# SamsungLabs/imvoxelnet

Hardware: AMD Instinct MI355X
Metric: images/sec/node (KITTI 3x384x1280, 216x248x12 vox) (higher is better)
Workload: dtype f32 (fp16 (hi, lo) pair MFMA operands: the Winograd-domain neck GEMMs and the chained 2-D trunk); 1 GPU; kitti_mono_1x3x384x1280_vox216x248x12_resnet50_fpn64_kittineck_anchor3dhead; batch_per_gpu=4, global_batch=4, parallelism=dp1, api=ImVoxelNet.simple_test(img, img_metas), detections_last_step=64

## Files before the change

imvoxelnet_amd/_lib.py:

```python
import ctypes as C
import os

_HERE = os.path.dirname(os.path.abspath(__file__))
LIB_PATH = os.environ.get('IVX_LIB_PATH') or os.path.join(_HERE, 'csrc', 'libimvoxel_hip.so')
_lib = None


class IvxError(RuntimeError):
    pass


class ConvDesc(C.Structure):
    _fields_ = [(n, C.c_int32) for n in
                ('B', 'D', 'H', 'W', 'Cin', 'Cout', 'KD', 'KH', 'KW', 'sd', 'sh', 'sw', 'pd', 'ph', 'pw',
                 'relu', 'res_mode', 'res_h', 'res_w', 'wgt_layout', 'out_mode', 'res_after_act')] + [('post_scale', C.c_float),
                                                                  ('in_dtype', C.c_int32), ('out_dtype', C.c_int32), ('res_scale', C.c_float),
                                                                  ('wino_operands', C.c_int32)]


class ConvRouteOpts(C.Structure):
    _fields_ = [(n, C.c_int32) for n in ('winograd', 'winograd_tile', 'wino_operands', 'split')] + [('winograd_min_pos', C.c_int64), ('winograd_2d_min_ch', C.c_int32)]


class ConvRoute(C.Structure):
# ... 66 lines not shown
                ('bytes', C.c_double), ('name', C.c_char * 48)]


class PlanInfo(C.Structure):
    _fields_ = [(n, C.c_int64) for n in ('cam_bytes', 'arena', 'ws_off', 'ws_bytes', 'ws2_off', 'ws2_bytes', 'total', 'scal_off', 'scal_bytes')] + \
               [(n, C.c_int32) for n in ('slot_bytes', 'n_sides', 's0', 's1', 'n_steps', 'n_tensors')]


class PlanStep(C.Structure):
    _fields_ = [(n, C.c_int32) for n in ('kind', 'in_', 'res', 'out', 'out2', 'fuse_out', 'fuse', 'side', 'join', 'tile', 'pio', 'amax_n', 'amax_in_n',
                                         'n_extra_in', 'n_extra_out')] + \
               [('extra_in', C.c_int32 * 12), ('extra_out', C.c_int32 * 4)] + \
               [(n, C.c_int64) for n in ('split', 'ws', 'amax_out', 'amax_in')] + [('name', C.c_char * 48)]


class PlanTensor(C.Structure):
    _fields_ = [(n, C.c_int64) for n in ('off', 'bytes', 'used', 'slot')] + \
               [(n, C.c_int32) for n in ('first', 'last', 'fmt', 'esz', 'caller_owned', 'boundary')]


class ImagePrepDesc(C.Structure):
    _fields_ = [(n, C.c_int32) for n in ('src_h', 'src_w', 'src_row_bytes', 'dst_h', 'dst_w', 'pad_h', 'pad_w', 'to_rgb')] + \
               [('mean', C.c_float * 3), ('std', C.c_float * 3)]


def declare_plan_view(L):
    key = [C.c_void_p, C.c_char_p, C.c_int32, C.c_int32, C.c_int32, C.c_int32]
    L.ivx_model_plan_info.argtypes = key + [C.POINTER(PlanInfo)]
    L.ivx_model_plan_step.argtypes = key + [C.c_int32, C.POINTER(PlanStep)]
    L.ivx_model_plan_tensor.argtypes = key + [C.c_int32, C.POINTER(PlanTensor)]


EXPORTS = ['ivx_model_plan_info', 'ivx_model_plan_step', 'ivx_model_plan_tensor', 'ivx_bottleneck_proj_supported', 'ivx_bottleneck_proj_pack', 'ivx_bottleneck_proj_fwd_pio', 'ivx_anchor_head_decode', 'ivx_fcos3d_head_decode', 'ivx_nms_rotated_bev', 'ivx_nms_aligned3d', 'ivx_bottleneck_supported', 'ivx_bottleneck_fwd_pio', 'ivx_amax_f32', 'ivx_stem_pool_filter_bytes', 'ivx_stem_pool_pack_filters', 'ivx_stem_pool_out_dims', 'ivx_stem_pool_fwd_pair', 'ivx_conv_winograd_set_variant', 'ivx_ubench_mfma', 'ivx_ubench_copy', 'ivx_version', 'ivx_last_error', 'ivx_conv_out_dims', 'ivx_conv_fwd', 'ivx_conv_fwd_naive', 'ivx_conv_set_tile_override', 'ivx_conv_set_epilogue_mode', 'ivx_conv_set_plan_mode', 'ivx_topk_set_mode', 'ivx_conv_workspace_bytes', 'ivx_conv_fwd_ws', 'ivx_conv_set_halo_mode', 'ivx_bf16_pair_split', 'ivx_f16_pair_split', 'ivx_conv_pair_supported', 'ivx_bf16_pair_pack_filters', 'ivx_conv_route', 'ivx_conv_pio_workspace_bytes', 'ivx_conv_fwd_pio', 'ivx_conv_fwd_pio_naive', 'ivx_pair_pack_filters', 'ivx_nchw_to_nhwc_amax', 'ivx_maxpool2d_fwd_pair', 'ivx_f16_pair_merge', 'ivx_model_calibrate_fp8', 'ivx_model_calibrate_fp8_ex', 'ivx_amax_bf16', 'ivx_conv_winograd_output_blocks', 'ivx_conv_winograd_issued_fraction', 'ivx_conv_winograd_output_amax', 'ivx_conv_winograd_input_amax', 'ivx_conv_winograd_fused_supported', 'ivx_conv_winograd_fused_blocks', 'ivx_conv_winograd_gemm_output_amax',
           'ivx_conv_winograd_supported', 'ivx_conv_winograd_weight_elems', 'ivx_conv_winograd_weights', 'ivx_conv_winograd_workspace_bytes',
           'ivx_conv_winograd_input', 'ivx_conv_winograd_gemm', 'ivx_conv_winograd_output', 'ivx_conv_winograd_fwd',
           'ivx_maxpool2d_fwd', 'ivx_maxpool2d_fwd_bf16', 'ivx_maxpool2d_fwd_fp8', 'ivx_global_avgpool_fwd', 'ivx_global_avgpool_fwd_bf16', 'ivx_upsample_trilinear2x_fwd', 'ivx_dcn_im2col_fwd', 'ivx_dcn_im2col_fwd_bf16', 'ivx_dcn_im2col_fwd_pair', 'ivx_nchw_to_nhwc', 'ivx_image_s2d_bf16', 'ivx_nhwc_to_nchw', 'ivx_backproject_mean_fwd', 'ivx_backproject_mean_fwd_amax', 'ivx_backproject_amax_blocks', 'ivx_backproject_mean_fwd_bf16', 'ivx_upsample_trilinear2x_fwd_bf16', 'ivx_backproject_sum_fwd', 'ivx_volume_normalize_fwd',
           'ivx_backproject_accum_fwd', 'ivx_backproject_accum_fwd_bf16', 'ivx_volume_mean_fwd', 'ivx_backproject_fwd_ex', 'ivx_backproject_gather_fwd',
           'ivx_anchor_head_workspace_bytes', 'ivx_anchor_head_get_bboxes', 'ivx_fcos_head_workspace_bytes',
           'ivx_fcos_head_level_candidates', 'ivx_nms_workspace_bytes',
           'ivx_nms_bev', 'ivx_boxes_overlap_bev', 'ivx_aligned_3d_nms', 'ivx_aligned_3d_nms_workspace_bytes', 'ivx_aligned_3d_nms_ws', 'ivx_multiclass_nms_workspace_bytes', 'ivx_multiclass_nms_bev',
           'ivx_create', 'ivx_destroy', 'ivx_weights_load', 'ivx_weights_finalize', 'ivx_model_workspace_bytes', 'ivx_model_forward',
           'ivx_backbone_fpn_workspace_bytes', 'ivx_backbone_fpn_fwd', 'ivx_neck3d_workspace_bytes', 'ivx_neck3d_out_dims',
           'ivx_neck3d_kitti_fwd', 'ivx_neck3d_nuscenes_fwd', 'ivx_neck3d_levels', 'ivx_neck3d_fast_fwd', 'ivx_neck3d_unet_fwd',
           'ivx_model_forward_levels', 'ivx_model_anchors', 'ivx_compute_projection', 'ivx_voxel_new_origin', 'ivx_fold_batchnorm',
           'ivx_model_trace', 'ivx_model_trace_count', 'ivx_model_trace_read',
           'ivx_model_detect_workspace_bytes', 'ivx_model_max_detections', 'ivx_model_detect', 'ivx_layout_head_decode', 'ivx_layout_extrinsics',
           'ivx_indoor_tail_workspace_bytes', 'ivx_indoor_tail_get_bboxes',
           'ivx_rescale_size', 'ivx_image_prep_u8',
           'ivx_kitti_image_box_overlap', 'ivx_kitti_compute_statistics', 'ivx_kitti_collect_scores', 'ivx_kitti_fused_statistics']


def lib():
    global _lib
    if _lib is not None:
        return _lib
    if not os.path.exists(LIB_PATH):
        raise IvxError(f'{LIB_PATH} is missing: build it with `python -m imvoxelnet_amd._build` '
                       '(or __graft_entry__.build()).  There is no CPU fallback.')
    L = C.CDLL(LIB_PATH)
    vp, i32, i64, f32 = C.c_void_p, C.c_int32, C.c_int64, C.c_float
    L.ivx_version.restype = C.c_int
    L.ivx_last_error.restype = C.c_char_p
    L.ivx_conv_out_dims.argtypes = [C.POINTER(ConvDesc), C.POINTER(i32), C.POINTER(i32), C.POINTER(i32)]
    for name in ('ivx_conv_fwd', 'ivx_conv_fwd_naive'):
        getattr(L, name).argtypes = [C.POINTER(ConvDesc), vp, vp, vp, vp, vp, vp, vp]
    L.ivx_conv_set_tile_override.argtypes = [C.c_int]
    L.ivx_conv_set_halo_mode.argtypes = [C.c_int]
    L.ivx_conv_set_epilogue_mode.argtypes = [C.c_int]
    L.ivx_conv_set_plan_mode.argtypes = [C.c_int]
    L.ivx_conv_winograd_output_blocks.argtypes = [C.POINTER(ConvDesc), i32]
    L.ivx_conv_winograd_output_blocks.restype = i32
    L.ivx_conv_winograd_output_amax.argtypes = [C.POINTER(ConvDesc), i32, vp, vp, vp, vp, vp, i64, vp, vp]
    L.ivx_conv_winograd_input_amax.argtypes = [C.POINTER(ConvDesc), i32, vp, vp, i64, vp, i32, vp]
    L.ivx_conv_winograd_fused_supported.argtypes = [C.POINTER(ConvDesc), i32]
    L.ivx_conv_winograd_fused_blocks.argtypes = [C.POINTER(ConvDesc), i32]
    L.ivx_conv_winograd_fused_blocks.restype = i32
    L.ivx_conv_winograd_gemm_output_amax.argtypes = [C.POINTER(ConvDesc), i32, vp, vp, vp, vp, vp, vp, i64, vp, vp]
    L.ivx_bf16_pair_split.argtypes = [vp, i64, vp, vp]
    L.ivx_f16_pair_split.argtypes = [vp, i64, f32, vp, vp]
    L.ivx_conv_pair_supported.argtypes = [C.POINTER(ConvDesc)]
    L.ivx_bf16_pair_pack_filters.argtypes = [vp, i32, i32, i32, i32, vp]
    L.ivx_conv_route.argtypes = [C.POINTER(ConvDesc), i32, C.POINTER(ConvRouteOpts), C.POINTER(ConvRoute)]
    L.ivx_conv_pio_workspace_bytes.argtypes = [C.POINTER(ConvDesc), C.POINTER(PairIO)]
    L.ivx_conv_pio_workspace_bytes.restype = i64
    L.ivx_amax_f32.argtypes = [vp, i64, vp, vp]
    L.ivx_stem_pool_filter_bytes.restype = i64
    L.ivx_stem_pool_filter_bytes.argtypes = []
    L.ivx_stem_pool_pack_filters.argtypes = [vp, vp, vp, vp]
    L.ivx_stem_pool_out_dims.argtypes = [i32, i32, C.POINTER(i32), C.POINTER(i32)]
    L.ivx_stem_pool_fwd_pair.argtypes = [vp, i32, i32, i32, vp, vp, vp, f32, f32, vp, vp, vp, vp, vp]
    L.ivx_bottleneck_supported.argtypes = [C.POINTER(BottleneckDesc)]
    L.ivx_bottleneck_fwd_pio.argtypes = [C.POINTER(BottleneckDesc), C.POINTER(BottleneckIO)] + [vp] * 12
    L.ivx_bottleneck_proj_supported.argtypes = [C.POINTER(BottleneckDesc), i32]
    L.ivx_bottleneck_proj_pack.argtypes = [vp, vp, vp, vp, vp, vp, i32, i32, vp, vp, vp, C.POINTER(f32), C.POINTER(f32), C.POINTER(f32)]
    L.ivx_bottleneck_proj_fwd_pio.argtypes = [C.POINTER(BottleneckDesc), i32, C.POINTER(BottleneckIO), f32] + [vp] * 12
    L.ivx_conv_fwd_pio.argtypes = [C.POINTER(ConvDesc), C.POINTER(PairIO), vp, vp, vp, vp, vp, vp, vp, i64, vp]
    L.ivx_conv_fwd_pio_naive.argtypes = [C.POINTER(ConvDesc), C.POINTER(PairIO), vp, vp, vp, vp, vp, vp, vp]
    L.ivx_pair_pack_filters.argtypes = [vp, i32, i32, i32, vp, vp, vp, vp, C.POINTER(f32), C.POINTER(f32)]
    L.ivx_nchw_to_nhwc_amax.argtypes = [vp, i32, i32, i64, i32, vp, vp, vp]
    L.ivx_maxpool2d_fwd_pair.argtypes = [vp, i32, i32, i32, i32, i32, i32, i32, vp, vp, f32, f32, vp, vp, vp]
    L.ivx_f16_pair_merge.argtypes = [vp, i64, vp, vp, vp]
    L.ivx_conv_workspace_bytes.argtypes = [C.POINTER(ConvDesc)]
    L.ivx_conv_workspace_bytes.restype = i64
    L.ivx_conv_fwd_ws.argtypes = [C.POINTER(ConvDesc), vp, vp, vp, vp, vp, vp, vp, i64, vp]
    D = C.POINTER(ConvDesc)
    L.ivx_conv_winograd_supported.argtypes = [D, i32]
    L.ivx_conv_winograd_issued_fraction.argtypes = [D]
    L.ivx_conv_winograd_issued_fraction.restype = C.c_float
    L.ivx_conv_winograd_weight_elems.argtypes = [D, i32]
    L.ivx_conv_winograd_weight_elems.restype = i64
# ... 107 lines not shown
```

imvoxelnet_amd/csrc/conv_igemm.hip:

```cpp
#include "ivx_common.h"
#include <stdlib.h>

#ifndef IVX_CONV_TU
#define IVX_CONV_TU 0
#endif
struct ConvParams;
struct ConvPlan;
int ivx_conv_launch_f32(ConvParams &p, const ConvPlan &pl, hipStream_t st);
int ivx_conv_launch_lowp(ConvParams &p, const ConvPlan &pl, hipStream_t st);
int ivx_conv_launch_pair_bf16(ConvParams &p, const ConvPlan &pl, hipStream_t st);
int ivx_conv_launch_pair_f16(ConvParams &p, const ConvPlan &pl, hipStream_t st);
int ivx_conv_launch_halo(ConvParams &p, int cfg, hipStream_t st);
int ivx_conv_launch_fold4(ConvParams &p, const IvxWinoFold &f, int n2, hipStream_t st);
int ivx_conv_fold4_blocks(long long M, int Cout);

typedef float f32x16 __attribute__((ext_vector_type(16)));
typedef float f32x4 __attribute__((ext_vector_type(4)));
typedef float f32x2 __attribute__((ext_vector_type(2)));
typedef __bf16 bf16x8 __attribute__((ext_vector_type(8)));
typedef _Float16 f16x8 __attribute__((ext_vector_type(8)));

struct ConvParams {
  const float *in, *wgt, *scale, *shift, *res;
  float *out;
  int B, D, H, W, Cin;
  int Cout, KD, KH, KW;
  int sd, sh, sw, pd, ph, pw;
  int Do, Ho, Wo;
  int M, K;
  int relu, res_mode, rH, rW;
  int kmode;
  int out_mode;
  int Cr;
  int res_after_act;
  float post_scale;
  int ksplit;
  float *partial;
  int q_total, q_begin, q_count, bm;
  int in_bf16;
  int out_bf16;
  long long g_in, g_w, g_out;
  int groups;
  int narrow_epilogue;
  int in_fp8;
  int out_fp8;
  float res_scale;
  int in_pair;
  int pio;
  const float *in_scale_p;
  int out_pair, res_pair;
  const float *res_scale_p;
  float *out_scale_p;
  const unsigned *amax_in, *amax_res;
  unsigned *amax_out;
  float wbound, sbound;
  const unsigned *cp_src;
  unsigned *cp_dst;
  int stagger_ticks, stagger_shift, stagger_first;
#ifdef IVX_CONV_TIMELINE
  unsigned long long *tl;
#endif
};

struct PairIO { float inv_in, inv_res, s_out; bool sat; float post; };
__device__ __forceinline__ PairIO conv_pair_io(const ConvParams &p) {
  PairIO io = {1.0f, 1.0f, 1.0f, false, p.post_scale};
  if (p.in_scale_p) io.inv_in = 1.0f / *p.in_scale_p;
  if (p.res_pair && p.res_scale_p) io.inv_res = 1.0f / *p.res_scale_p;
  if (p.out_pair) {
    const int lane = threadIdx.x & 63;
    float a = p.amax_in ? __uint_as_float(p.amax_in[lane]) : 0.f;
    float r = (p.amax_res && p.res_mode) ? __uint_as_float(p.amax_res[lane]) : 0.f;
#pragma unroll
    for (int o = 32; o > 0; o >>= 1) {
      a = fmaxf(a, __shfl_xor(a, o));
      r = fmaxf(r, __shfl_xor(r, o));
    }
    const float bound = (a * p.wbound + p.sbound + r) * fabsf(p.post_scale) * 1.001f;
    io.s_out = ivx_pow2_scale(bound);
    io.sat = !(bound < 3.0e38f);
    if (io.sat) io.s_out = 0.00390625f;
  }
  return io;
}
__device__ __forceinline__ size_t pair_off(size_t row, int n, int C) { return row * (size_t)(2 * C) + (size_t)((n >> 4) * 32 + (n & 15)); }

struct fp8_t { unsigned char v; };
typedef long i64_t;

__device__ __forceinline__ float fp8_to_f32(unsigned char b) { return __builtin_amdgcn_cvt_f32_fp8((int)b, 0); }
// ... 1166 lines not shown
    IVX_REQUIRE(!(d->res_mode && io->res_dtype == IVX_F16_PAIR) || (d->Cout % 16 == 0 && io->res_scale), "ivx_conv_fwd_pio: a pair residual needs Cout %% 16 == 0 and res_scale");
  }
  IVX_REQUIRE(!pair || (d->Cin % 16 == 0 && d->out_mode == 0), "ivx_conv_fwd: bf16-pair input needs Cin %% 16 == 0 and out_mode 0");
  IVX_REQUIRE(d->in_dtype != IVX_FP8 || d->Cin % 16 == 0, "ivx_conv_fwd: fp8 input needs Cin %% 16 == 0");
  IVX_REQUIRE((d->in_dtype != IVX_FP8 && d->out_dtype != IVX_FP8) || d->out_mode == 0, "ivx_conv_fwd: fp8 is built for out_mode 0 only");
  const int ck = d->in_dtype == IVX_FP8 ? 128 : (d->in_dtype == IVX_BF16 ? 64 : 32);
  IVX_REQUIRE(d->wgt_layout == 0 || (d->wgt_layout == 1 && d->Cin % ck == 0),
              "ivx_conv_fwd: wgt_layout 1 needs Cin %% %d == 0 (128-byte channel chunks)", ck);
  IVX_REQUIRE(d->in_dtype == IVX_F32 || d->Cin % 8 == 0, "ivx_conv_fwd: bf16 input needs Cin %% 8 == 0");
  IVX_REQUIRE(d->res_mode == 0 || res, "ivx_conv_fwd: res_mode set but res is NULL");
  if (d->res_mode == 2) {
    IVX_REQUIRE(Do == 1 && d->res_h > 0 && d->res_w > 0, "ivx_conv_fwd: res_mode 2 needs a 2-D output and res dims");
  }
  p->in = (const float *)in; p->wgt = (const float *)wgt; p->scale = scale; p->shift = shift;
  p->res = d->res_mode ? (const float *)res : nullptr; p->out = (float *)out;
  p->in_bf16 = d->in_dtype == IVX_BF16 || pair; p->out_bf16 = d->out_dtype == IVX_BF16;
  p->in_pair = d->in_dtype == IVX_BF16_PAIR ? 1 : (d->in_dtype == IVX_F16_PAIR ? 2 : 0);
  p->in_fp8 = d->in_dtype == IVX_FP8; p->out_fp8 = d->out_dtype == IVX_FP8;
  p->res_scale = d->res_scale == 0.f ? 1.0f : d->res_scale;
  p->B = d->B; p->D = d->D; p->H = d->H; p->W = d->W; p->Cin = cin_el;
  p->Cout = d->Cout; p->KD = d->KD; p->KH = d->KH; p->KW = d->KW;
  p->sd = d->sd; p->sh = d->sh; p->sw = d->sw; p->pd = d->pd; p->ph = d->ph; p->pw = d->pw;
  p->Do = Do; p->Ho = Ho; p->Wo = Wo; p->M = (int)M; p->K = (int)K;
  p->relu = d->relu; p->res_mode = d->res_mode; p->rH = d->res_h; p->rW = d->res_w; p->kmode = d->wgt_layout;
  p->out_mode = d->out_mode; p->Cr = d->out_mode == 1 ? d->Cout / 8 : d->Cout; p->res_after_act = d->res_after_act;
  p->post_scale = d->post_scale == 0.f ? 1.0f : d->post_scale;
  p->ksplit = 1; p->partial = nullptr; p->q_total = 0; p->q_begin = 0; p->q_count = 0; p->bm = 0;
  p->stagger_ticks = 0; p->stagger_shift = 0; p->stagger_first = 0;
  p->groups = 1; p->g_in = p->g_w = p->g_out = 0;
  p->narrow_epilogue = g_narrow_epilogue;
#ifdef IVX_CONV_TIMELINE
  p->tl = g_timeline;
#endif
  p->cp_src = nullptr; p->cp_dst = nullptr;
  p->pio = 0; p->in_scale_p = nullptr; p->out_pair = 0; p->res_pair = 0; p->res_scale_p = nullptr; p->out_scale_p = nullptr;
  p->amax_in = p->amax_res = nullptr; p->amax_out = nullptr; p->wbound = 0.f; p->sbound = 0.f;
  if (io) {
    p->pio = 1;
    p->in_scale_p = io->in_scale;
    p->out_pair = d->out_dtype == IVX_F16_PAIR; p->out_bf16 = 0;
    p->res_pair = d->res_mode && io->res_dtype == IVX_F16_PAIR;
    p->res_scale_p = io->res_scale; p->out_scale_p = p->out_pair ? io->out_scale : nullptr;
    p->amax_in = io->amax_in; p->amax_res = d->res_mode ? io->amax_res : nullptr; p->amax_out = io->amax_out;
    p->wbound = io->wbound; p->sbound = io->sbound;
  }
  return IVX_OK;
}

extern "C" int ivx_conv_out_dims(const ivx_conv_desc *d, int32_t *Do, int32_t *Ho, int32_t *Wo) {
  IVX_REQUIRE(d && Do && Ho && Wo, "ivx_conv_out_dims: null argument");
  const int od = (d->D + 2 * d->pd - d->KD) / d->sd + 1;
  const int oh = (d->H + 2 * d->ph - d->KH) / d->sh + 1;
  const int ow = (d->W + 2 * d->pw - d->KW) / d->sw + 1;
  IVX_REQUIRE(d->D + 2 * d->pd >= d->KD && d->H + 2 * d->ph >= d->KH && d->W + 2 * d->pw >= d->KW && od > 0 && oh > 0 && ow > 0,
              "ivx_conv_out_dims: kernel larger than padded input");
  *Do = od; *Ho = oh; *Wo = ow;
  return IVX_OK;
}

template <int TM, int TN, int WR, int WC>
static void launch_cfg(const ConvParams &p, hipStream_t st) {
  constexpr int BM = WR * TM * 32, BN = WC * TN * 32;
  dim3 grid((p.M + BM - 1) / BM, (p.Cout + BN - 1) / BN);
  hipLaunchKernelGGL((conv_igemm_f32_kernel<TM, TN, WR, WC>), grid, dim3(256), 0, st, p);
}

#endif
// ... 285 lines not shown
      ivx_set_error("ivx_conv_fwd: tile %d has no pair-operand instantiation (61, 63, 66, 67, 73 .. 77, 81 .. 83, 85, 166, 174, 177, 179, 183; fp16 pairs also 474, 475, 574)", pl.cfg);
      return IVX_ERR_INVALID_ARG;
  }
  return IVX_OK;
}

#if IVX_CONV_TU == 3
int ivx_conv_launch_pair_bf16(ConvParams &p, const ConvPlan &pl, hipStream_t st) { return launch_pair<1>(p, pl, st); }
#else
int ivx_conv_launch_pair_f16(ConvParams &p, const ConvPlan &pl, hipStream_t st) { return launch_pair<2>(p, pl, st); }
#endif
#endif

#if IVX_CONV_TU == 5
template <typename T, int TM, int TN, int WR, int WC, int WPE, int PAIR, int NBUF, int TAIL = 1, int SW = 1, int ZR = 0, int DI = 0>
__global__ __launch_bounds__(64 * WR * WC, WPE) void conv_wino_halo_kernel(const ConvParams p, const unsigned in_bytes, const unsigned w_bytes) {
  constexpr int BM = WR * TM * 32, BN = WC * TN * 32, NT = 64 * WR * WC;
  constexpr int BK = 32, EPC = 8, NCH = 4, RP = NT / NCH;
  static_assert((SW * BM) % RP == 0 && (3 * BN) % RP == 0, "A rows and the three taps of B rows in whole passes (+ one 16-row tail pass of A)");
  static_assert(SW == 1 || TAIL == 0, "the stride-2 form uses overlapping tiles");
  static_assert(!DI || SW == 2, "de-interleaved staging is the stride-2 form's");
  constexpr int APASS = SW * BM / RP, AROWS = SW * BM + 16 * TAIL;
  constexpr int BMO = TAIL ? BM : (SW == 1 ? BM - 2 - ZR : BM - 1);
  constexpr int ZROW = TAIL ? BM + 2 : SW * BM - 1;
  constexpr int BPASS = 3 * BN / RP;
  constexpr int BUF = (AROWS + 3 * BN) * BK;
  constexpr int D = NBUF - 1;
  constexpr int LPG = APASS + BPASS;
  static_assert((D - 1) * (LPG + TAIL) <= 15, "vmcnt immediate");
  __shared__ __attribute__((aligned(16))) T smem[NBUF * BUF];
  static_assert(sizeof(smem) >= (size_t)NT / 64 * 4096, "4 KB of staging LDS per wave for the transposed epilogue");
  const int tid = threadIdx.x, lane = tid & 63, wid = tid >> 6;
  const int wr = wid / WC, wc = wid % WC;
  int mt, nt;
  {
    const int Nt = (p.Cout + BN - 1) / BN;
    const int xcd = blockIdx.x & 7, idx = blockIdx.x >> 3;
    const int lt = idx / Nt;
    nt = idx - lt * Nt;
    mt = xcd * p.q_total + lt;
  }
  if (mt * BMO >= p.M) return;
  const int m0 = mt * BMO, n0 = nt * BN;
  const size_t gz = blockIdx.z;
  if (p.cp_dst && blockIdx.x == 0 && blockIdx.z == 0 && tid == 0) *p.cp_dst = *p.cp_src;
#ifdef IVX_CONV_TIMELINE
  const unsigned long long tl0 = __builtin_amdgcn_s_memrealtime();
  unsigned long long tl1 = 0, tl2 = 0;
#endif
  const __amdgpu_buffer_rsrc_t rs_in =
      __builtin_amdgcn_make_buffer_rsrc((void *)((const char *)p.in + gz * (size_t)p.g_in * sizeof(T)), 0, in_bytes, 0x00020000);
  const __amdgpu_buffer_rsrc_t rs_w =
      __builtin_amdgcn_make_buffer_rsrc((void *)((const char *)p.wgt + gz * (size_t)p.g_w * sizeof(T)), 0, w_bytes, 0x00020000);
  const int lr = tid / NCH;
  const int cc = (tid & (NCH - 1)) ^ ((lr >> 2) & 3);
  const int wid_u = __builtin_amdgcn_readfirstlane(wid);
  const unsigned OOB = 0x80000000u;
  typedef __attribute__((address_space(3))) void *lds_ptr_t;
  unsigned a_base[APASS + 1];
  a_base[APASS] = OOB;
#pragma unroll
  for (int j = 0; j < APASS + TAIL; ++j) {
    const int li = j < APASS ? lr + RP * j : BM + (lane >> 2);
    const int row = SW * m0 - 1 + (DI ? (li < BM ? 2 * li : 2 * (li - BM) + 1) : li);
    const bool zr = ZR && !TAIL && li == ZROW;
    a_base[j] = (row >= 0 && row < SW * p.M && (j < APASS || (lane >> 2) < 2) && !zr) ? ((unsigned)row * (unsigned)p.Cin + cc * EPC) * (unsigned)sizeof(T) : OOB;
  }
  unsigned b_base[BPASS];
#pragma unroll
  for (int j = 0; j < BPASS; ++j) {
    const int r = lr + RP * j, tap = r / BN, n = n0 + (r - tap * BN);
    b_base[j] = n < p.Cout ? ((unsigned)n * (unsigned)p.K + tap * 64 + cc * EPC) * (unsigned)sizeof(T) : OOB;
  }
  const int G = p.Cin / BK;
  auto load_group = [&](int g, int buf) {
    T *Ab = smem + buf * BUF + wid_u * (64 / NCH) * BK;
    T *Bb = Ab + AROWS * BK;
    const unsigned ka = (unsigned)g * BK * (unsigned)sizeof(T);
    const unsigned kb = ((unsigned)(g >> 1) * 3u * 64u + (unsigned)(g & 1) * 32u) * (unsigned)sizeof(T);
#pragma unroll
    for (int j = 0; j < APASS; ++j) {
      const unsigned vo = a_base[j] == OOB ? OOB : a_base[j] + ka;
      __builtin_amdgcn_raw_ptr_buffer_load_lds(rs_in, (lds_ptr_t)(Ab + RP * j * BK), 16, vo, 0, 0, 0);
    }
    if (TAIL && wid_u == 0) {
      const unsigned vo = a_base[APASS] == OOB ? OOB : a_base[APASS] + ka;
      __builtin_amdgcn_raw_ptr_buffer_load_lds(rs_in, (lds_ptr_t)(smem + buf * BUF + BM * BK), 16, vo, 0, 0, 0);
    }
#pragma unroll
    for (int j = 0; j < BPASS; ++j) {
      const unsigned vo = b_base[j] == OOB ? OOB : b_base[j] + kb;
      __builtin_amdgcn_raw_ptr_buffer_load_lds(rs_w, (lds_ptr_t)(Bb + RP * j * BK), 16, vo, 0, 0, 0);
    }
  };
  const int rl = lane & 31, fh = lane >> 5;
  bool ok0[TM], ok2[TM];
#pragma unroll
  for (int i = 0; i < TM; ++i) {
    const int z = (m0 + (wr * TM + i) * 32 + rl) % p.Wo;
// ... 65 lines not shown
        const T *rowp = Bc + (kz * BN + j * 32 + rl) * BK;
        bh[j] = *reinterpret_cast<const f32x4 *>(rowp + ((fh ^ bsw) * EPC));
        bl[j] = *reinterpret_cast<const f32x4 *>(rowp + (((2 + fh) ^ bsw) * EPC));
      }
      if (!ZR && kz != 1) {
#pragma unroll
        for (int i = 0; i < TM; ++i) {
          const bool ok = kz == 0 ? ok0[i] : ok2[i];
          ah[i] = ok ? ah[i] : zero4;
          al[i] = ok ? al[i] : zero4;
        }
      }
#pragma unroll
      for (int i = 0; i < TM; ++i)
#pragma unroll
        for (int j = 0; j < TN; ++j) {
          acc[i][j] = pair_mfma<PAIR>(ah[i], bh[j], acc[i][j]);
          acc[i][j] = pair_mfma<PAIR>(ah[i], bl[j], acc[i][j]);
          acc[i][j] = pair_mfma<PAIR>(al[i], bh[j], acc[i][j]);
        }
    }
    cur = cur + 1 == NBUF ? 0 : cur + 1;
    nxt = nxt + 1 == NBUF ? 0 : nxt + 1;
  }
#ifdef IVX_CONV_TIMELINE
  tl2 = __builtin_amdgcn_s_memrealtime();
#endif
  __syncthreads();
  if constexpr (TAIL) {
    conv_epilogue_wide<TM, TN>(p, acc, m0, n0, wr, wc, lane, reinterpret_cast<float *>(smem) + wid_u * 1024, gz * (size_t)p.g_out);
  } else {
    float *stage = reinterpret_cast<float *>(smem) + wid_u * 1024;
    float *outp = p.out + gz * (size_t)p.g_out;
    const int mlim = (m0 + BMO < p.M) ? m0 + BMO : p.M;
    const int col_l = lane & 31, hh = lane >> 5, rrow = lane >> 3, c4 = (lane & 7) * 4;
#pragma unroll
    for (int j = 0; j < TN; ++j) {
      const int nb = n0 + (wc * TN + j) * 32 + c4;
      const bool nok = nb < p.Cout;
#pragma unroll
      for (int i = 0; i < TM; ++i) {
#pragma unroll
        for (int r = 0; r < 16; ++r) stage[((r & 3) + 8 * (r >> 2) + 4 * hh) * 32 + col_l] = acc[i][j][r];
        const int mb = m0 + (wr * TM + i) * 32 + rrow;
#pragma unroll
        for (int q = 0; q < 4; ++q) {
          const f32x4 v = *reinterpret_cast<const f32x4 *>(stage + (rrow + 8 * q) * 32 + c4);
          const int m = mb + 8 * q;
          if (m < mlim && nok) *reinterpret_cast<f32x4 *>(outp + (size_t)m * p.Cout + nb) = v;
        }
      }
    }
  }
#ifdef IVX_CONV_TIMELINE
  if (p.tl && tid == 0) {
    unsigned long long *t = p.tl + ((size_t)blockIdx.z * gridDim.x + blockIdx.x) * 8;
    t[0] = tl0; t[1] = tl1; t[2] = tl2; t[3] = __builtin_amdgcn_s_memrealtime();
    t[4] = __builtin_amdgcn_s_getreg(63492); t[5] = __builtin_amdgcn_s_getreg(63508);
  }
#endif
}

template <int TM, int TN, int WR, int WC, int WPE, int PAIR, int NBUF, int TAIL = 1, int SW = 1, int ZR = 0, int DI = 0>
static void launch_halo(ConvParams &p, hipStream_t st) {
  constexpr int BM = (WR * TM * 32) - (TAIL ? 0 : (SW == 1 ? 2 + ZR : 1)), BN = WC * TN * 32;
  const int64_t in_bytes = (int64_t)p.B * p.D * p.H * p.W * p.Cin * 2, w_bytes = (int64_t)p.Cout * p.K * 2;
  const long long Mt = (p.M + BM - 1) / BM, Nt = (p.Cout + BN - 1) / BN;
  p.bm = BM;
  p.q_total = (int)((Mt + 7) / 8); p.q_begin = 0; p.q_count = p.q_total;
  const dim3 grid((unsigned)(8LL * p.q_total * Nt), 1, p.groups > 1 ? p.groups : 1);
  auto kern = conv_wino_halo_kernel<__bf16, TM, TN, WR, WC, WPE, PAIR, NBUF, TAIL, SW, ZR, DI>;
  hipLaunchKernelGGL(kern, grid, dim3(64 * WR * WC), 0, st, p, (unsigned)in_bytes, (unsigned)w_bytes);
}

template <typename T, int Z, int WCOL, int WN, int WPE, int PAIR, int SW = 1>
__global__ __launch_bounds__(64 * WCOL * (Z / 3) * WN, WPE) void conv_wino_zblk_kernel(const ConvParams p, const unsigned in_bytes, const unsigned w_bytes) {
  static_assert(Z == 3 || Z == 6, "three output z-blocks per wave");
  constexpr int ZI = SW * Z;
  constexpr int ZH = Z / 3, NW = WCOL * ZH * WN, NT = 64 * NW;
  constexpr int CT = WCOL * 32, AR = ZI * CT, BN = WN * 32;
  constexpr int NS = 2 * SW + 3;
  constexpr int BK = 32, EPC = 8, NCH = 4, RP = NT / NCH;
  constexpr int APASS = (AR + RP - 1) / RP, BPASS = (3 * BN + RP - 1) / RP;
  static_assert(AR % 16 == 0 && (3 * BN) % 16 == 0, "a wave's 16 rows of a pass are inside or outside as a whole");
  constexpr int BUF = (AR + 3 * BN) * BK;
  __shared__ __attribute__((aligned(16))) T smem[2 * BUF];
  static_assert(sizeof(smem) >= (size_t)NW * 4096, "4 KB of staging LDS per wave for the transposed epilogue");
  const int tid = threadIdx.x, lane = tid & 63, wid = tid >> 6;
  const int wid_u = __builtin_amdgcn_readfirstlane(wid);
  const int cg = wid_u / (ZH * WN), zh = (wid_u / WN) % ZH, nb = wid_u % WN;
  int mt, nt;
  {
    const int Nt = (p.Cout + BN - 1) / BN;
    const int xcd = blockIdx.x & 7, idx = blockIdx.x >> 3;
    const int lt = idx / Nt;
    nt = idx - lt * Nt;
    mt = xcd * p.q_total + lt;
  }
  const int c0 = mt * CT, n0 = nt * BN;
  const int m0 = c0 * Z;
  if (m0 >= p.M) return;
#ifdef IVX_CONV_TIMELINE
  const unsigned long long tl0 = __builtin_amdgcn_s_memrealtime();
  unsigned long long tl1 = 0, tl2 = 0;
#endif
  const size_t gz = blockIdx.z;
  if (p.cp_dst && blockIdx.x == 0 && blockIdx.z == 0 && tid == 0) *p.cp_dst = *p.cp_src;
  const __amdgpu_buffer_rsrc_t rs_in =
      __builtin_amdgcn_make_buffer_rsrc((void *)((const char *)p.in + gz * (size_t)p.g_in * sizeof(T)), 0, in_bytes, 0x00020000);
  const __amdgpu_buffer_rsrc_t rs_w =
      __builtin_amdgcn_make_buffer_rsrc((void *)((const char *)p.wgt + gz * (size_t)p.g_w * sizeof(T)), 0, w_bytes, 0x00020000);
  const int lr = tid / NCH;
  const int cc = (tid & (NCH - 1)) ^ ((lr >> 2) & 3);
  const unsigned OOB = 0x80000000u;
  typedef __attribute__((address_space(3))) void *lds_ptr_t;
  unsigned a_base[APASS], b_base[BPASS];
#pragma unroll
  for (int j = 0; j < APASS; ++j) {
    const int li = lr + RP * j;
    const int z = li / CT, c = li - z * CT;
    const int row = (c0 + c) * ZI + z;
    a_base[j] = (li < AR && row < SW * p.M) ? ((unsigned)row * (unsigned)p.Cin + cc * EPC) * (unsigned)sizeof(T) : OOB;
  }
#pragma unroll
  for (int j = 0; j < BPASS; ++j) {
    const int r = lr + RP * j, tap = r / BN, n = n0 + (r - tap * BN);
    b_base[j] = (r < 3 * BN && n < p.Cout) ? ((unsigned)n * (unsigned)p.K + tap * 64 + cc * EPC) * (unsigned)sizeof(T) : OOB;
  }
  const int G = p.Cin / BK;
  auto load_group = [&](int g, int buf) {
    T *Ab = smem + buf * BUF + wid_u * (64 / NCH) * BK;
    T *Bb = Ab + AR * BK;
    const unsigned ka = (unsigned)g * BK * (unsigned)sizeof(T);
    const unsigned kb = ((unsigned)(g >> 1) * 3u * 64u + (unsigned)(g & 1) * 32u) * (unsigned)sizeof(T);
#pragma unroll
    for (int j = 0; j < APASS; ++j) {
      if (RP * j + wid_u * 16 < AR) {
        const unsigned vo = a_base[j] == OOB ? OOB : a_base[j] + ka;
        __builtin_amdgcn_raw_ptr_buffer_load_lds(rs_in, (lds_ptr_t)(Ab + RP * j * BK), 16, vo, 0, 0, 0);
      }
    }
#pragma unroll
    for (int j = 0; j < BPASS; ++j) {
      if (RP * j + wid_u * 16 < 3 * BN) {
        const unsigned vo = b_base[j] == OOB ? OOB : b_base[j] + kb;
        __builtin_amdgcn_raw_ptr_buffer_load_lds(rs_w, (lds_ptr_t)(Bb + RP * j * BK), 16, vo, 0, 0, 0);
      }
    }
  };
  const int rl = lane & 31, fh = lane >> 5, sw = (rl >> 2) & 3;
  const int z0 = zh * 3;
  f32x16 acc[3];
#pragma unroll
  for (int i = 0; i < 3; ++i)
#pragma unroll
// ... 23 lines not shown
    for (int kz = 0; kz < 3; ++kz) {
      const T *rowp = B0 + kz * BN * BK;
      const f32x4 bh = *reinterpret_cast<const f32x4 *>(rowp + ((fh ^ sw) * EPC));
      const f32x4 bl = *reinterpret_cast<const f32x4 *>(rowp + (((2 + fh) ^ sw) * EPC));
#pragma unroll
      for (int zo = 0; zo < 3; ++zo) {
        const int zs = SW * (z0 + zo) + kz - 1;
        if (zs >= 0 && zs < ZI) {
          acc[zo] = pair_mfma<PAIR>(ah[SW * zo + kz], bh, acc[zo]);
          acc[zo] = pair_mfma<PAIR>(ah[SW * zo + kz], bl, acc[zo]);
          acc[zo] = pair_mfma<PAIR>(al[SW * zo + kz], bh, acc[zo]);
        }
      }
    }
    cur ^= 1;
  }
#ifdef IVX_CONV_TIMELINE
  tl2 = __builtin_amdgcn_s_memrealtime();
#endif
  __syncthreads();
  float *stage = reinterpret_cast<float *>(smem) + wid_u * 1024;
  float *outp = p.out + gz * (size_t)p.g_out;
  const int col_l = lane & 31, hh = lane >> 5, rrow = lane >> 3, c4 = (lane & 7) * 4;
  const int nbc = n0 + nb * 32 + c4;
  const bool nok = nbc < p.Cout;
#pragma unroll
  for (int zo = 0; zo < 3; ++zo) {
#pragma unroll
    for (int r = 0; r < 16; ++r) stage[((r & 3) + 8 * (r >> 2) + 4 * hh) * 32 + col_l] = acc[zo][r];
#pragma unroll
    for (int q = 0; q < 4; ++q) {
      const f32x4 v = *reinterpret_cast<const f32x4 *>(stage + (rrow + 8 * q) * 32 + c4);
      const int m = m0 + (cg * 32 + rrow + 8 * q) * Z + z0 + zo;
      if (m < p.M && nok) *reinterpret_cast<f32x4 *>(outp + (size_t)m * p.Cout + nbc) = v;
    }
  }
#ifdef IVX_CONV_TIMELINE
  if (p.tl && tid == 0) {
    unsigned long long *t = p.tl + ((size_t)blockIdx.z * gridDim.x + blockIdx.x) * 8;
    t[0] = tl0; t[1] = tl1; t[2] = tl2; t[3] = __builtin_amdgcn_s_memrealtime();
    t[4] = __builtin_amdgcn_s_getreg(63492); t[5] = __builtin_amdgcn_s_getreg(63508);
  }
#endif
}

template <int Z, int WCOL, int WN, int WPE, int SW = 1>
static void launch_zblk(ConvParams &p, hipStream_t st) {
  constexpr int AR = Z * WCOL * 32, BN = WN * 32;
  const int64_t in_bytes = (int64_t)p.B * p.D * p.H * p.W * p.Cin * 2, w_bytes = (int64_t)p.Cout * p.K * 2;
  const long long Mt = (p.M + AR - 1) / AR, Nt = (p.Cout + BN - 1) / BN;
  p.bm = AR;
  p.q_total = (int)((Mt + 7) / 8); p.q_begin = 0; p.q_count = p.q_total;
  const dim3 grid((unsigned)(8LL * p.q_total * Nt), 1, p.groups > 1 ? p.groups : 1);
  auto kern = conv_wino_zblk_kernel<__bf16, Z, WCOL, WN, WPE, 2, SW>;
  hipLaunchKernelGGL(kern, grid, dim3(64 * WCOL * (Z / 3) * WN), 0, st, p, (unsigned)in_bytes, (unsigned)w_bytes);
}

static int zblk_wrong_z(int want, int got) {
  ivx_set_error("ivx_conv_launch_halo: this z-blocked config is built for columns of %d slices, the layer has %d", want, got);
  return IVX_ERR_INVALID_ARG;
}

int ivx_conv_launch_halo(ConvParams &p, int cfg, hipStream_t st) {
  if (p.in_pair != 2) {
    ivx_set_error("ivx_conv_launch_halo: fp16 pair operands only");
    return IVX_ERR_INVALID_ARG;
  }
// ... 485 lines not shown
    if (!launch) continue;
    if (pl.ws_bytes > 0 && (!workspace || workspace_bytes < pl.ws_bytes)) {
      ivx_set_error("%s: workspace too small (%lld < %lld); size it with ivx_conv_workspace_bytes", who, (long long)workspace_bytes,
                    (long long)pl.ws_bytes);
      return IVX_ERR_WORKSPACE;
    }
    const int rc = run_conv(q, pl, workspace, st);
    if (rc != IVX_OK) return rc;
  }
  return IVX_OK;
}

extern "C" int ivx_conv_fwd(const ivx_conv_desc *d, const void *in, const void *wgt, const float *scale,
                            const float *shift, const void *res, void *out, ivx_stream_t stream) {
  ConvParams p;
  int rc = fill_params(d, in, wgt, scale, shift, res, out, &p);
  if (rc != IVX_OK) return rc;
  int64_t need;
  rc = conv_dispatch(p, false, true, nullptr, 0, (hipStream_t)stream, &need, "ivx_conv_fwd");
  if (rc != IVX_OK) return rc;
  IVX_CHECK_LAUNCH("ivx_conv_fwd");
  return IVX_OK;
}

static bool zblk_rule(const ConvParams &p) { return p.Wo == 3 && p.W == 3 && p.Cout > 64; }

extern "C" float ivx_conv_winograd_issued_fraction(const ivx_conv_desc *d) {
  if (!d || d->wino_operands != IVX_F16_PAIR || d->KW != 3 || d->sw != 1 || d->pw != 1 || d->W != 3 || d->Cin % 64 || d->Cout <= 64 || d->wgt_layout != 1 ||
      g_halo_mode >= 0 || g_tile_override != 0)
    return 1.0f;
  return 7.0f / 9.0f;
}

int ivx_conv_grouped_launch(const ivx_conv_desc *d, int groups, const float *in, long long g_in, const float *wgt, long long g_w,
                            float *out, long long g_out, hipStream_t st, const unsigned *cp_src, unsigned *cp_dst) {
  ConvParams p;
  int rc = fill_params(d, in, wgt, nullptr, nullptr, nullptr, out, &p);
  if (rc != IVX_OK) return rc;
  IVX_REQUIRE(groups >= 1 && groups <= 65535, "ivx_conv_grouped_launch: bad group count");
  IVX_REQUIRE((d->in_dtype == IVX_F32 || d->in_dtype == IVX_BF16_PAIR || d->in_dtype == IVX_F16_PAIR) && d->out_dtype == IVX_F32 &&
                  d->out_mode == 0 && d->res_mode == 0,
              "ivx_conv_grouped_launch: fp32 or pair operands, plain fp32 output only");
  if (!dma_applicable(p)) {
    ivx_set_error("ivx_conv_grouped_launch: one group must stay below 2 GiB");
    return IVX_ERR_UNSUPPORTED;
  }
  if (cp_dst && !p.in_pair) {
    if (hipMemcpyAsync(cp_dst, cp_src, 4, hipMemcpyDeviceToDevice, st) != hipSuccess) {
      ivx_set_error("ivx_conv_grouped_launch: hipMemcpyAsync failed");
      return IVX_ERR_HIP;
    }
  } else {
    p.cp_src = cp_src; p.cp_dst = cp_dst;
  }
  p.groups = groups; p.g_in = g_in; p.g_w = g_w; p.g_out = g_out;
  if (p.in_pair == 2 && p.kmode == 1 && d->KD == 1 && d->KH == 1 && d->KW == 3 && d->sw == 2 && d->pw == 1 && p.W == 2 * p.Wo && p.Cin % 64 == 0 &&
      ((g_halo_mode >= 21 && g_halo_mode < 30) || (g_halo_mode >= 40 && g_halo_mode < 50) || g_halo_mode >= 70 || (g_halo_mode < 0 && g_tile_override == 0))) {
    return ivx_conv_launch_halo(p, g_halo_mode >= 21 ? g_halo_mode : 42, st);
  }
  if (p.in_pair == 2 && p.kmode == 1 && d->KD == 1 && d->KH == 1 && d->KW == 3 && d->sw == 1 && d->pw == 1 && p.Cin % 64 == 0 &&
      ((g_halo_mode > 0 && g_halo_mode < 21) || (g_halo_mode >= 30 && g_halo_mode < 40) || (g_halo_mode >= 50 && g_halo_mode < 70) ||
       (g_halo_mode < 0 && g_tile_override == 0))) {
    static const int halo_small = getenv("IVX_HALO_SMALL") ? atoi(getenv("IVX_HALO_SMALL")) : 1;
    const bool few = halo_small && p.Cout > 64 && !zblk_rule(p) && (long long)((p.M + 252) / 253) * ((p.Cout + 127) / 128) * groups < 512;
    const int cfg = g_halo_mode > 0 ? g_halo_mode : ((p.Cout <= 64 || few) ? 30 : (zblk_rule(p) ? 50 : 33));
    return ivx_conv_launch_halo(p, cfg, st);
  }
  ConvPlan pl = {g_tile_override, 1, 1, 0, 0, 0, 0};
  if (pl.cfg == 0 && p.in_pair) {
    pl.cfg = p.Cout <= 64 ? 76 : (p.Cout <= 128 ? 81 : (p.in_pair == 2 && p.kmode == 1 ? 183 : 82));
    const long long nblk = (long long)groups * ((p.M + 127) / 128) * ((p.Cout + 127) / 128);
    if (nblk < 2500) pl.cfg = 67;
  }
  if (pl.cfg == 0) {
    const long long nblk = (long long)groups * ((p.M + 127) / 128) * ((p.Cout + 127) / 128);
    if (p.Cout <= 32) pl.cfg = 44;
    else if (nblk >= 2500) pl.cfg = p.Cout > 64 ? (p.Cout == 128 && p.K == 384 ? 58 : 54) : 49;
    else pl.cfg = p.K <= 640 ? 47 : 46;
  }
  TileInfo t;
  if (!tile_info(pl.cfg, &t) || (pl.cfg >= 61) != (p.in_pair != 0)) {
    ivx_set_error("ivx_conv_grouped_launch: tile %d does not match the operand type", pl.cfg);
    return IVX_ERR_INVALID_ARG;
  }
  return launch_one(p, pl, st);
}

int ivx_conv_grouped_fold4(const ivx_conv_desc *d, int groups, const float *in, long long g_in, const float *wgt, long long g_w, const IvxWinoFold *f,
                           hipStream_t st) {
  ConvParams p;
  float dummy;
  int rc = fill_params(d, in, wgt, nullptr, nullptr, nullptr, &dummy, &p);
  if (rc != IVX_OK) return rc;
  IVX_REQUIRE(d->in_dtype == IVX_F16_PAIR && d->KD == 1 && d->KH == 1 && d->KW == 3 && d->sw == 1 && d->pw == 1 && d->wgt_layout == 1 && f && f->out,
              "ivx_conv_grouped_fold4: fp16 pair operands, 1x1x3 along z with stride 1 and padding 1, chunk-major filters");
  p.groups = groups; p.g_in = g_in; p.g_w = g_w; p.g_out = 0;
  return ivx_conv_launch_fold4(p, *f, groups, st);
}

// ... 81 lines not shown
```

imvoxelnet_amd/csrc/model.cpp:

```cpp
#include <hip/hip_runtime_api.h>
#include <math.h>
#include <stdarg.h>
#include <string.h>

#include <algorithm>
#include <cstdlib>
#include <map>
#include <memory>
#include <string>
#include <vector>

#include "../../include/imvoxel.h"
#include "../../include/imvoxel_lab.h"

void ivx_set_error(const char *fmt, ...);

#define M_REQUIRE(cond, ...)        \
  do {                              \
    if (!(cond)) {                  \
      ivx_set_error(__VA_ARGS__);   \
      return IVX_ERR_INVALID_ARG;   \
    }                               \
  } while (0)
#define M_HIP(call, what)                                                        \
  do {                                                                           \
    hipError_t e_ = (call);                                                      \
    if (e_ != hipSuccess) {                                                      \
      ivx_set_error("%s: %s", what, hipGetErrorString(e_));                      \
      return IVX_ERR_HIP;                                                        \
    }                                                                            \
  } while (0)
#define M_TRY(call)                 \
  do {                              \
    int rc_ = (call);               \
    if (rc_ != IVX_OK) return rc_;  \
  } while (0)

namespace {

inline int64_t align256(int64_t v) { return (v + 255) / 256 * 256; }

inline uint16_t f32_to_f16_bits(float f) {
  uint32_t x;
  memcpy(&x, &f, 4);
  const uint32_t sign = (x >> 16) & 0x8000u, ax = x & 0x7fffffffu;
  if (ax >= 0x7f800000u) return (uint16_t)(sign | (ax > 0x7f800000u ? 0x7e00u : 0x7c00u));
  if (ax < 0x38800000u) {
    float a;
// ... 78 lines not shown

struct Step {
  StepKind kind;
  int layer = -1;
  int in = -1, res = -1, out = -1, out2 = -1;
  int res_mode = 0;
  int res_after_act = 0;
  float post_scale = 1.0f;
  int aux = 0;
};

struct TInfo {
  int B = 0, D = 0, H = 0, W = 0, C = 0;
  int64_t bytes = 0, off = -1;
  int first = -1, last = -1;
  bool raw = false;
  int esz = 4;
  int fmt = 0;
  int64_t slot = -1;
  int64_t elems() const { return (int64_t)B * D * H * W * C; }
};

struct PlanStep {
  ivx_conv_desc d;
  int tile = 0;
  int64_t ws = 0;
  int64_t amax_out = -1, amax_in = -1;
  int amax_n = 0, amax_in_n = 0;
  int pio = 0;
  int64_t split = 0;
  int bound_layer = -1;
  int fuse = 0, fuse_out = -1;
  int side = 0, join = 0;
};

struct Plan {
  std::vector<TInfo> t;
  std::vector<PlanStep> ps;
  int64_t arena = 0, ws_off = 0, ws_bytes = 0, tail_ws = 0, total = 0;
  ivx_anchor_head_desc tail;
  int64_t cam_bytes = 0, cam_proj = 0, cam_origin = 0, cam_crop = 0, cam_lvl_vs[3] = {0, 0, 0}, cam_lvl_no[3] = {0, 0, 0};
  int n_views = 1;
  ivx_indoor_tail_desc itail;
  int max_det = 0;
  int64_t scal_off = 0, scal_bytes = 0;
  int64_t ws2_off = 0, ws2_bytes = 0;
  int n_sides = 0;
  int s0 = 0, s1 = 0;
};

}

struct ivx_model {
  ivx_model_cfg cfg;
  std::vector<ConvLayer> layers;
  std::vector<Step> steps;
  int n_tensors = 0;
  int trunk0 = 0, trunk1 = 0, lift_step = -1, neck0 = 0, neck1 = 0, head_step = -1, tail_step = -1;
  int t_img = -1, t_fpn0 = -1, t_volume = -1, t_valid = -1, t_neck = -1, t_head = -1;
  std::vector<int> t_levels;
  int head0 = -1;
  std::vector<int> t_headout, t_cb, t_cs, t_cc;
  float head_scales[3] = {1.f, 1.f, 1.f};
  int t_c5 = -1, t_angle = -1, t_layout = -1, layout_step = -1;
  std::vector<std::vector<char>> cam_ring;
  size_t cam_next = 0;
  std::map<std::string, HostTensor> weights;
  bool finalized = false;
  std::vector<float> anchors_host;
  int anchors_h = 0, anchors_w = 0;
  float *anchors_dev = nullptr;
  size_t anchors_cap = 0;
  std::vector<float> anchors_given;
  std::map<std::string, std::unique_ptr<Plan>> plans;
  std::vector<void *> owned;
  std::vector<float> pack_a, pack_b;
  bool fp8_on = false;
  float *calib_dev = nullptr;
  bool trace_on = false;
  bool trace_skip = false;
  int trace_level = 2;
  struct TraceRec { int step, stage, is3d; double flops, bytes; hipEvent_t e0, e1; std::string name; };
  std::vector<TraceRec> trace;
  std::vector<hipEvent_t> event_pool;
  size_t events_used = 0;
  hipStream_t side = nullptr;
  hipEvent_t ev_fork = nullptr;
  std::vector<hipEvent_t> ev_join;
};

namespace {

int new_tensor(ivx_model *m) { return m->n_tensors++; }

int add_conv(ivx_model *m, ConvLayer L, int in, int res = -1, int res_mode = 0) {
  m->layers.push_back(std::move(L));
  Step s;
  s.kind = ST_CONV;
  s.layer = (int)m->layers.size() - 1;
  s.in = in;
  s.res = res;
  s.res_mode = res >= 0 ? (res_mode ? res_mode : 1) : 0;
  s.out = new_tensor(m);
  m->steps.push_back(s);
  return s.out;
}

ConvLayer conv2d(const std::string &name, int cin, int cout, int k, int stride, int pad, bool relu, const std::string &w,
                 const std::string &b, const std::string &bn) {
  ConvLayer L;
  L.name = name; L.dims = 2; L.cin = cin; L.cout = cout;
  L.k[0] = 1; L.k[1] = k; L.k[2] = k;
  L.s[0] = 1; L.s[1] = stride; L.s[2] = stride;
  L.p[0] = 0; L.p[1] = pad; L.p[2] = pad;
  L.relu = relu; L.w_keys = {w}; L.b_keys = {b}; L.bn = bn;
// ... 884 lines not shown
    }
  }
  for (int i = r.s0; i < r.s1; ++i) {
    const Step &s = m->steps[i];
    PlanStep &pc = pl->ps[i];
    if (s.kind != ST_CONV || pc.tile == 0 || pc.d.wino_operands != IVX_F16_PAIR) continue;
    for (int j = i - 1; j >= r.s0; --j) {
      const Step &q = m->steps[j];
      if (q.out != s.in) continue;
      PlanStep &pp = pl->ps[j];
      if (q.kind == ST_LIFT && m->cfg.sampling == IVX_SAMPLE_NEAREST) {
        const TInfo &vol = pl->t[q.out];
        const int32_t nb = ivx_backproject_amax_blocks(vol.B, n_views, vol.D, vol.H, vol.W);
        if (nb > 0) {
          if (pp.amax_out < 0) { pp.amax_out = top; pp.amax_n = nb; top += align256((int64_t)nb * 4); }
          pc.amax_in = pp.amax_out;
          pc.amax_in_n = pp.amax_n;
        }
      }
      if (q.kind == ST_CONV && pp.tile > 0) {
        if (pp.amax_out < 0) {
          const int32_t nb = ivx_conv_winograd_output_blocks(&pp.d, pp.tile);
          M_REQUIRE(nb > 0, "layer %s: %s", m->layers[q.layer].name.c_str(), ivx_last_error());
          pp.amax_out = top;
          pp.amax_n = nb;
          top += align256((int64_t)nb * 4);
        }
        pc.amax_in = pp.amax_out;
        pc.amax_in_n = pp.amax_n;
      }
      break;
    }
  }
  if (n_slots > 0) {
    top = align256(top);
    pl->scal_off = top;
    pl->scal_bytes = (int64_t)n_slots * 512;
    top += pl->scal_bytes;
  }
  pl->arena = align256(top);
  pl->ws_off = pl->arena;
  pl->ws_bytes = align256(pl->ws_bytes);
  pl->total = pl->arena + pl->ws_bytes;
  if (pl->n_sides > 0) {
    for (int i = r.s0; i < r.s1; ++i)
      if (pl->ps[i].side > 0) pl->ws2_bytes = std::max(pl->ws2_bytes, pl->ps[i].ws);
    pl->ws2_bytes = align256(pl->ws2_bytes);
    pl->ws2_off = pl->total;
    pl->total += pl->ws2_bytes;
  }
  return IVX_OK;
}

std::string plan_key(const char *what, int B, int V, int H, int W) {
  char buf[96];
  snprintf(buf, sizeof(buf), "%s:%d:%d:%d:%d", what, B, V, H, W);
  return buf;
}

TInfo tinfo(int B, int D, int H, int W, int C, int esz = 4) {
  TInfo t; t.B = B; t.D = D; t.H = H; t.W = W; t.C = C; t.esz = esz; t.bytes = align256(t.elems() * esz);
  return t;
}

int get_plan(ivx_model *m, const char *what, Range r, int B, int V, int H, int W, const std::map<int, TInfo> &inputs, Plan **out,
             hipStream_t stream) {
// ... 64 lines not shown
  }
  if (!m->anchors_dev) {
    void *p = nullptr;
    M_HIP(hipMalloc(&p, std::max<size_t>(n, 1) * sizeof(float)), "hipMalloc (anchors)");
    m->owned.push_back(p);
    m->anchors_dev = (float *)p;
    m->anchors_cap = n;
  }
  M_HIP(hipMemcpyAsync(m->anchors_dev, m->anchors_host.data(), n * sizeof(float), hipMemcpyHostToDevice, st), "hipMemcpyAsync (anchors)");
  M_HIP(hipStreamSynchronize(st), "hipStreamSynchronize (anchors)");
  m->anchors_h = d.H; m->anchors_w = d.W;
  return IVX_OK;
}

int run_steps(ivx_model *m, const Plan &pl, Range r, const Bind &bd, void *workspace, int64_t workspace_bytes, hipStream_t st,
              const char *who) {
  M_REQUIRE(workspace && ((uintptr_t)workspace & 255) == 0, "%s: workspace must be non-null and 256-byte aligned", who);
  if (workspace_bytes < pl.total) {
    ivx_set_error("%s: workspace too small (%lld < %lld); size it with the matching *_workspace_bytes call", who, (long long)workspace_bytes,
                  (long long)pl.total);
    return IVX_ERR_WORKSPACE;
  }
  char *base = (char *)workspace;
  void *ws = base + pl.ws_off;
  auto ptr = [&](int t) -> void * {
    auto it = bd.ext.find(t);
    if (it != bd.ext.end()) return it->second;
    return base + pl.t[t].off;
  };
  auto slotp = [&](int t) -> uint32_t * { return (t >= 0 && pl.t[t].slot >= 0) ? (uint32_t *)(base + pl.scal_off + pl.t[t].slot * 512) : nullptr; };
  auto scalep = [&](int t) -> float * { uint32_t *q = slotp(t); return q ? (float *)(q + IVX_AMAX_SLOTS) : nullptr; };
  if (pl.scal_bytes > 0 && r.s0 <= m->trunk0 && r.s1 > m->trunk0)
    M_HIP(hipMemsetAsync(base + pl.scal_off, 0, (size_t)pl.scal_bytes, st), "hipMemsetAsync (amax slots)");
  const bool span2d = m->trace_on && m->trace_level == 1 && m->cfg.with_trunk;
  std::vector<char> forked((size_t)std::max(pl.n_sides, 1), 0);
  double span_flops = 0.0, span_bytes = 0.0;
  for (int i = r.s0; i < r.s1; ++i) {
    const Step &s = m->steps[i];
    const TInfo &in = pl.t[s.in];
    const bool in_span = span2d && i >= m->trunk0 && i < m->trunk1;
    if (in_span && i == m->trunk0) M_TRY(trace_begin(m, i, 6, 0, 0.0, 0.0, "2-D trunk (ResNet-50 + FPN level 0)", st));
    const bool was_on = m->trace_on;
    if (in_span) {
      m->trace_on = false;
      {
        const PlanStep &ps = pl.ps[i];
        auto tb = [&](int t) { return t >= 0 ? (double)pl.t[t].elems() * pl.t[t].esz : 0.0; };
        if (s.kind == ST_CONV && ps.fuse != 2) {
          const ConvLayer &L = m->layers[s.layer];
          if (ps.fuse == 1) {
            const ConvLayer &L2 = m->layers[m->steps[i + 1].layer], &L3 = m->layers[m->steps[i + 2].layer];
            span_bytes += tb(s.in) + tb(ps.fuse_out) + 4.0 * ((double)L.cout * L.cin + 9.0 * L2.cout * L2.cin + (double)L3.cout * L3.cin);
          } else if (ps.fuse == 5) {
            const ConvLayer &L2 = m->layers[m->steps[i + 1].layer], &L3 = m->layers[m->steps[i + 2].layer];
            span_bytes += tb(s.in) + tb(ps.fuse_out) + 4.0 * ((double)L.cout * L.cin + 9.0 * L2.cout * L2.cin + (double)L3.cout * (L3.cin + L.cin));
          } else {
            span_bytes += tb(s.in) + tb(s.out) + tb(s.res) + (double)pl.t[s.in].esz * L.cout * L.cin_pad * L.k[0] * L.k[1] * L.k[2];
          }
        } else if (s.kind == ST_MAXPOOL && ps.fuse == 4) {
          span_bytes += tb(s.out) + tb(m->t_img);
        } else if (s.kind == ST_IMG2CL && ps.fuse == 3) {
          span_bytes += tb(s.in);
        } else if (s.kind != ST_CONV && s.kind != ST_LAYOUT) {
          span_bytes += tb(s.in) + tb(s.out) + tb(s.res);
        }
      }
// ... 102 lines not shown
        const void *res = s.res >= 0 ? ptr(s.res) : nullptr;
        const TInfo &o = pl.t[s.out];
        const int is3d = in.D > 1 && in.W > 1;
        hipStream_t cst = st;
        void *cws = ws;
        int64_t cws_bytes = pl.ws_bytes;
        if (ps.side > 0 && !(m->trace_on && m->trace_level != 3) && pl.ws2_off > 0) {
          if (!m->side) {
            M_HIP(hipStreamCreateWithFlags(&m->side, hipStreamNonBlocking), "hipStreamCreateWithFlags");
            M_HIP(hipEventCreateWithFlags(&m->ev_fork, hipEventDisableTiming), "hipEventCreateWithFlags");
          }
          while ((int)m->ev_join.size() < pl.n_sides) {
            hipEvent_t e;
            M_HIP(hipEventCreateWithFlags(&e, hipEventDisableTiming), "hipEventCreateWithFlags");
            m->ev_join.push_back(e);
          }
          M_HIP(hipEventRecord(m->ev_fork, st), "hipEventRecord");
          M_HIP(hipStreamWaitEvent(m->side, m->ev_fork, 0), "hipStreamWaitEvent");
          cst = m->side;
          cws = base + pl.ws2_off;
          cws_bytes = pl.ws2_bytes;
          forked[ps.side - 1] = 1;
        }
        if (ps.join > 0 && forked[ps.join - 1]) {
          M_HIP(hipStreamWaitEvent(st, m->ev_join[ps.join - 1], 0), "hipStreamWaitEvent");
          forked[ps.join - 1] = 0;
        }
        if (ps.tile && m->trace_on) {
          const int n = ps.tile + 2, tiles = o.B * ((ps.d.D + 2 * ps.d.pd - 2 + ps.tile - 1) / ps.tile) * ((ps.d.H + 2 * ps.d.ph - 2 + ps.tile - 1) / ps.tile);
          int32_t zo_d, zo_h, zo;
          M_TRY(ivx_conv_out_dims(&ps.d, &zo_d, &zo_h, &zo));
          const double vb = 4.0 * n * n * tiles * ps.d.W * ps.d.Cin, mb = 4.0 * n * n * tiles * zo * ps.d.Cout;
          M_TRY(trace_begin(m, i, 1, is3d, 0.0, 4.0 * in.elems() + vb, L.name, st));
          M_TRY(ivx_conv_winograd_input_amax(&ps.d, ps.tile, ptr(s.in), ws, pl.ws_bytes, ps.amax_in >= 0 ? (const float *)(base + ps.amax_in) : nullptr,
                                             ps.amax_in_n, st));
          M_TRY(trace_end(m, st));
          M_TRY(trace_begin(m, i, 2, is3d, (ps.d.wino_operands ? 3.0 : 1.0) * ivx_conv_winograd_issued_fraction(&ps.d) * 2.0 * n * n * tiles * zo * ps.d.Cout * ps.d.KW * ps.d.Cin,
                            vb + mb, L.name, st));
          M_TRY(ivx_conv_winograd_gemm(&ps.d, ps.tile, L.u.at(ps.tile * 8 + ps.d.wino_operands), ws, pl.ws_bytes, st));
          M_TRY(trace_end(m, st));
          M_TRY(trace_begin(m, i, 3, is3d, 0.0, mb + 4.0 * o.elems() * (res ? 2 : 1), L.name, st));
          M_TRY(ivx_conv_winograd_output_amax(&ps.d, ps.tile, L.scale, L.shift, res, ptr(s.out), ws, pl.ws_bytes,
                                              ps.amax_out >= 0 ? (float *)(base + ps.amax_out) : nullptr, st));
          M_TRY(trace_end(m, st));
          break;
        }
        M_TRY(trace_begin(m, i, 0, is3d, ((ps.pio || ps.split) ? 3.0 : 1.0) * 2.0 * o.elems() * L.cin * L.k[0] * L.k[1] * L.k[2], 0.0, L.name, st));
        if (ps.pio) {
          ivx_pair_io io;
          memset(&io, 0, sizeof(io));
          io.in_scale = scalep(s.in);
          io.res_dtype = s.res >= 0 ? pl.t[s.res].fmt : 0;
          io.res_scale = io.res_dtype == IVX_F16_PAIR ? scalep(s.res) : nullptr;
          io.out_scale = scalep(s.out);
          io.amax_in = slotp(s.in); io.amax_res = slotp(s.res); io.amax_out = slotp(s.out);
          io.wbound = L.wbound; io.sbound = L.sbound;
          M_TRY(ivx_conv_fwd_pio(&ps.d, &io, ptr(s.in), L.wpair, L.scale_p, L.shift, res, ptr(s.out), cws, cws_bytes, cst));
        } else if (ps.tile) {
          M_TRY(ivx_conv_winograd_input_amax(&ps.d, ps.tile, ptr(s.in), ws, pl.ws_bytes, ps.amax_in >= 0 ? (const float *)(base + ps.amax_in) : nullptr,
                                             ps.amax_in_n, st));
          M_TRY(ivx_conv_winograd_gemm(&ps.d, ps.tile, L.u.at(ps.tile * 8 + ps.d.wino_operands), ws, pl.ws_bytes, st));
          M_TRY(ivx_conv_winograd_output_amax(&ps.d, ps.tile, L.scale, L.shift, res, ptr(s.out), ws, pl.ws_bytes,
                                              ps.amax_out >= 0 ? (float *)(base + ps.amax_out) : nullptr, st));
        } else if (m->fp8_on && L.fp8_eff) {
          M_TRY(ivx_conv_fwd_ws(&ps.d, ptr(s.in), L.fp8_eff >= 2 ? L.wq : L.w, L.scale_q, L.shift_q, res, ptr(s.out), cws, cws_bytes, cst));
        } else if (ps.split) {
          M_TRY(ivx_bf16_pair_split((const float *)ptr(s.in), in.elems(), cws, cst));
          M_TRY(ivx_conv_fwd_ws(&ps.d, cws, L.wsplit, L.scale, L.shift, res, ptr(s.out), (char *)cws + ps.split, cws_bytes - ps.split, cst));
        } else {
          M_TRY(ivx_conv_fwd_ws(&ps.d, ptr(s.in), L.w, L.scale, L.shift, res, ptr(s.out), cws, cws_bytes, cst));
          if (m->calib_dev && (L.fp8_eff == 1 || L.fp8_eff == 2))
            M_TRY(ivx_amax_bf16(ptr(s.out), o.elems(), m->calib_dev + s.layer, st));
        }
        M_TRY(trace_end(m, st));
        if (cst != st) M_HIP(hipEventRecord(m->ev_join[ps.side - 1], cst), "hipEventRecord");
        break;
      }
      case ST_LIFT: {
        M_REQUIRE(bd.proj && bd.new_origin && bd.crop, "%s: proj / new_origin / crop_hw are required", who);
        const TInfo &o = pl.t[s.out];
        M_TRY(trace_begin(m, i, 4, 1, 0.0, (double)in.esz * in.elems() + (double)o.esz * o.elems() + (double)o.elems() / o.C, "unprojection", st));
        if (m->cfg.sampling != IVX_SAMPLE_NEAREST) {
          ivx_backproject_desc ld = {};
          ld.B = o.B; ld.V = bd.V; ld.FH = in.H; ld.FW = in.W; ld.C = in.C; ld.X = o.D; ld.Y = o.H; ld.Z = o.W;
          for (int a = 0; a < 3; ++a) ld.voxel_size[a] = m->cfg.voxel_size[a];
          ld.feat_dtype = m->cfg.storage == IVX_BF16 ? IVX_BF16 : IVX_F32;
          ld.mode = IVX_LIFT_MEAN;
          ld.sampling = m->cfg.sampling;
          M_TRY(ivx_backproject_fwd_ex(&ld, ptr(s.in), bd.proj, bd.new_origin, bd.crop, ptr(s.out), nullptr, nullptr, (uint8_t *)ptr(s.out2), st));
          M_TRY(trace_end(m, st));
          break;
        }
        if (m->cfg.storage == IVX_BF16) {
          if (bd.V == 1 && in.C % 8 == 0)
            M_TRY(ivx_backproject_mean_fwd((const float *)ptr(s.in), o.B, 1, in.H, in.W, in.C / 2, bd.proj, bd.new_origin, bd.crop, m->cfg.voxel_size, o.D,
                                           o.H, o.W, (float *)ptr(s.out), (uint8_t *)ptr(s.out2), st));
          else
            M_TRY(ivx_backproject_mean_fwd_bf16(ptr(s.in), o.B, bd.V, in.H, in.W, in.C, bd.proj, bd.new_origin, bd.crop, m->cfg.voxel_size, o.D, o.H, o.W,
                                                ptr(s.out), (uint8_t *)ptr(s.out2), st));
          M_TRY(trace_end(m, st));
          break;
        }
        M_TRY(ivx_backproject_mean_fwd_amax((const float *)ptr(s.in), o.B, bd.V, in.H, in.W, in.C, bd.proj, bd.new_origin, bd.crop, m->cfg.voxel_size,
                                            o.D, o.H, o.W, (float *)ptr(s.out), (uint8_t *)ptr(s.out2),
                                            pl.ps[i].amax_out >= 0 ? (float *)(base + pl.ps[i].amax_out) : nullptr, st));
        M_TRY(trace_end(m, st));
        break;
      }
      case ST_DCN_COL: {
        const TInfo &om = pl.t[s.res];
        M_TRY(trace_begin(m, i, 0, 0, 0.0, (double)pl.t[s.out].esz * pl.t[s.out].elems(), "dcn columns", st));
        if (pl.ps[i].pio)
          M_TRY(ivx_dcn_im2col_fwd_pair(ptr(s.in), scalep(s.in), (const float *)ptr(s.res), in.B, in.H, in.W, in.C, 3, 3, s.aux, 1, 1, om.C,
                                        ptr(s.out), scalep(s.out), slotp(s.out), st));
        else if (m->cfg.storage == IVX_BF16)
          M_TRY(ivx_dcn_im2col_fwd_bf16(ptr(s.in), (const float *)ptr(s.res), in.B, in.H, in.W, in.C, 3, 3, s.aux, 1, 1, om.C, ptr(s.out), st));
        else
          M_TRY(ivx_dcn_im2col_fwd((const float *)ptr(s.in), (const float *)ptr(s.res), in.B, in.H, in.W, in.C, 3, 3, s.aux, 1, 1, om.C,
                                   (float *)ptr(s.out), st));
        M_TRY(trace_end(m, st));
        break;
      }
      case ST_AVGPOOL:
        if (m->cfg.storage == IVX_BF16)
          M_TRY(ivx_global_avgpool_fwd_bf16(ptr(s.in), in.B, (int64_t)in.D * in.H * in.W, in.C, (float *)ptr(s.out), st));
        else
          M_TRY(ivx_global_avgpool_fwd((const float *)ptr(s.in), in.B, (int64_t)in.D * in.H * in.W, in.C, (float *)ptr(s.out), st));
        break;
      case ST_LAYOUT: {
        if (!bd.metas && r.s1 == m->trunk1) break;
        M_REQUIRE(bd.metas && bd.proj_dev, "%s: a handle with a LayoutHead runs through ivx_model_detect (the projection is built from its angles)", who);
        const int B = in.B;
        std::vector<float> a((size_t)B * 2), l((size_t)B * 7), pj((size_t)B * 12);
        M_HIP(hipMemcpyAsync(a.data(), ptr(s.in), a.size() * 4, hipMemcpyDeviceToHost, st), "hipMemcpyAsync (angles)");
        M_HIP(hipMemcpyAsync(l.data(), ptr(s.res), l.size() * 4, hipMemcpyDeviceToHost, st), "hipMemcpyAsync (layout)");
        M_HIP(hipStreamSynchronize(st), "hipStreamSynchronize (LayoutHead)");
        for (int b = 0; b < B; ++b) {
          float ang[2], E[16];
          M_TRY(ivx_layout_head_decode(&a[(size_t)b * 2], &l[(size_t)b * 7], ang, bd.layout_host ? bd.layout_host + (size_t)b * 7 : nullptr));
// ... 586 lines not shown
        proj[(size_t)v * 12 + i * 4 + j] = acc;
      }
  }
  return IVX_OK;
}

extern "C" int ivx_voxel_new_origin(const float *origin, const int32_t *n_voxels, const float *voxel_size, float *new_origin) {
  M_REQUIRE(origin && n_voxels && voxel_size && new_origin, "ivx_voxel_new_origin: null argument");
  for (int a = 0; a < 3; ++a) {
    const float half = (float)n_voxels[a] / 2.0f;
    const float ext = half * voxel_size[a];
    new_origin[a] = origin[a] - ext;
  }
  return IVX_OK;
}

extern "C" int ivx_model_trace(ivx_model *m, int32_t enable) {
  M_REQUIRE(m, "ivx_model_trace: null handle");
  m->trace.clear();
  m->events_used = 0;
  m->trace_on = enable != 0;
  if (enable >= 1 && enable <= 3) m->trace_level = enable;
  return IVX_OK;
}

extern "C" int32_t ivx_model_trace_count(ivx_model *m) { return m ? (int32_t)m->trace.size() : -1; }

extern "C" int ivx_model_trace_read(ivx_model *m, int32_t i, ivx_trace_rec *rec) {
  M_REQUIRE(m && rec && i >= 0 && i < (int32_t)m->trace.size(), "ivx_model_trace_read: bad index");
  const ivx_model::TraceRec &r = m->trace[i];
  float ms = 0.f, start = 0.f;
  M_HIP(hipEventElapsedTime(&ms, r.e0, r.e1), "hipEventElapsedTime (synchronise the stream first)");
  M_HIP(hipEventElapsedTime(&start, m->trace[0].e0, r.e0), "hipEventElapsedTime");
  rec->step = r.step; rec->stage = r.stage; rec->is3d = r.is3d; rec->ms = ms; rec->start_ms = start; rec->flops = r.flops; rec->bytes = r.bytes;
  snprintf(rec->name, sizeof(rec->name), "%s", r.name.c_str());
  return IVX_OK;
}

static int plan_lookup(ivx_model *m, const char *what, int B, int V, int H, int W, const char *who, const Plan **pl) {
  M_REQUIRE(m && what, "%s: null argument", who);
  auto it = m->plans.find(plan_key(what, B, V, H, W));
  M_REQUIRE(it != m->plans.end(), "%s: no cached plan \"%s\" for (%d, %d, %d, %d); call the matching *_workspace_bytes first", who, what, B, V, H, W);
  *pl = it->second.get();
  return IVX_OK;
}

extern "C" int ivx_model_plan_info(ivx_model *m, const char *what, int32_t B, int32_t V, int32_t H, int32_t W, ivx_plan_info *info) {
  const Plan *pl;
  M_TRY(plan_lookup(m, what, B, V, H, W, "ivx_model_plan_info", &pl));
  M_REQUIRE(info, "ivx_model_plan_info: null argument");
  memset(info, 0, sizeof(*info));
  info->cam_bytes = pl->cam_bytes; info->arena = pl->arena; info->ws_off = pl->ws_off; info->ws_bytes = pl->ws_bytes;
  info->ws2_off = pl->ws2_off; info->ws2_bytes = pl->ws2_bytes; info->total = pl->total;
  info->scal_off = pl->scal_off; info->scal_bytes = pl->scal_bytes; info->slot_bytes = 512;
  info->n_sides = pl->n_sides; info->s0 = pl->s0; info->s1 = pl->s1;
  info->n_steps = (int32_t)m->steps.size(); info->n_tensors = m->n_tensors;
  return IVX_OK;
}

extern "C" int ivx_model_plan_step(ivx_model *m, const char *what, int32_t B, int32_t V, int32_t H, int32_t W, int32_t step, ivx_plan_step *rec) {
  const Plan *pl;
  M_TRY(plan_lookup(m, what, B, V, H, W, "ivx_model_plan_step", &pl));
  M_REQUIRE(rec && step >= pl->s0 && step < pl->s1, "ivx_model_plan_step: step %d is outside the plan's range [%d, %d)", step, pl->s0, pl->s1);
  const Step &s = m->steps[step];
  const PlanStep &ps = pl->ps[step];
  memset(rec, 0, sizeof(*rec));
  rec->kind = (int32_t)s.kind;
// ... 150 lines not shown
```

imvoxelnet_amd/csrc/winograd.hip:

```cpp
#include "ivx_common.h"
#include <stdlib.h>
int ivx_conv_launch_fold4w(const _Float16 *V, long long vs, const _Float16 *U, long long us, int M, int Cin_stored, int Cout, int Z, const IvxWinoFold &f,
                           hipStream_t st);

int ivx_conv_grouped_launch(const ivx_conv_desc *d, int groups, const float *in, long long g_in, const float *wgt, long long g_w,
                            float *out, long long g_out, hipStream_t st, const unsigned *cp_src, unsigned *cp_dst);
int ivx_conv_grouped_fold4(const ivx_conv_desc *d, int groups, const float *in, long long g_in, const float *wgt, long long g_w, const IvxWinoFold *f,
                           hipStream_t st);
int ivx_conv_fold4_blocks(long long M, int Cout);

namespace {

struct WinoP {
  const float *in, *scale, *shift, *res;
  float *out;
  float *V, *Mw;
  long long vs, ms;
  int B, X, Y, Z, C;
  int Xo, Yo, Zo, Co;
  int TX, TY;
  int px, py;
  int relu, res_mode, res_after_act;
  float post_scale;
  float *pmax;
  const unsigned *hdr;
#ifdef IVX_CONV_TIMELINE
  unsigned long long *tl;
#endif
};
#ifdef IVX_CONV_TIMELINE
#define WINO_TL_BEGIN const unsigned long long wtl0 = __builtin_amdgcn_s_memrealtime();
#define WINO_TL_END(p)                                                                                              \
  if ((p).tl && threadIdx.x == 0) {                                                                                \
    unsigned long long *t_ = (p).tl + (size_t)blockIdx.x * 8;                                                       \
    t_[0] = wtl0; t_[1] = wtl0; t_[2] = wtl0; t_[3] = __builtin_amdgcn_s_memrealtime();                             \
    t_[4] = __builtin_amdgcn_s_getreg(63492); t_[5] = __builtin_amdgcn_s_getreg(63508);                             \
  }
#else
#define WINO_TL_BEGIN
#define WINO_TL_END(p)
#endif

__device__ __forceinline__ bool wino_amax_bad(const float amax) { return !(amax < 3.0e38f); }
__device__ __forceinline__ float wino_pow2_scale(const float amax, const float gain_log2) {
  if (wino_amax_bad(amax)) return 0.00390625f;
  if (!(amax > 0.f)) return 1.0f;
  int e;
  (void)frexpf(amax, &e);
  int k = 15 - (int)gain_log2 - e;
  k = k < -120 ? -120 : (k > 120 ? 120 : k);
  return ldexpf(1.0f, k);
}
__device__ __forceinline__ float wino_pair_vscale(const unsigned *hdr) { return wino_pow2_scale(__uint_as_float(hdr[0]), 8.f); }
__device__ __forceinline__ float wino_mscale(const unsigned *hdr) { return hdr ? 1.0f / (wino_pair_vscale(hdr) * __uint_as_float(hdr[1])) : 1.0f; }

__device__ __forceinline__ float vabsmax(const float v) { return fabsf(v); }
__device__ __forceinline__ float vabsmax(const float2 v) { return fmaxf(fabsf(v.x), fabsf(v.y)); }
__device__ __forceinline__ float vabsmax(const float4 v) { return fmaxf(fmaxf(fabsf(v.x), fabsf(v.y)), fmaxf(fabsf(v.z), fabsf(v.w))); }
// ... 170 lines not shown
    u[3] = (1.0f / 90.0f) * g[0] + (1.0f / 45.0f) * g[1] + (2.0f / 45.0f) * g[2];
    u[4] = (1.0f / 90.0f) * g[0] - (1.0f / 45.0f) * g[1] + (2.0f / 45.0f) * g[2];
    u[5] = (32.0f / 45.0f) * g[0] + (16.0f / 45.0f) * g[1] + (8.0f / 45.0f) * g[2];
    u[6] = (32.0f / 45.0f) * g[0] - (16.0f / 45.0f) * g[1] + (8.0f / 45.0f) * g[2];
    u[7] = g[2];
  }
};

typedef _Float16 wf16x2 __attribute__((ext_vector_type(2)));
typedef unsigned u32x2w __attribute__((ext_vector_type(2)));
__device__ __forceinline__ float wino_sat16(const float x) {
  return (x > 65504.f && x < __builtin_inff()) ? 65504.f : ((x < -65504.f && x > -__builtin_inff()) ? -65504.f : x);
}
__device__ __forceinline__ void wino_pair2(const float2 v, const float s, unsigned *hi, unsigned *lo, const bool sat = false) {
  float x0 = v.x * s, x1 = v.y * s;
  if (sat) { x0 = wino_sat16(x0); x1 = wino_sat16(x1); }
  wf16x2 h, l;
  h[0] = (_Float16)x0;
  h[1] = (_Float16)x1;
  l[0] = (_Float16)(x0 - (float)h[0]);
  l[1] = (_Float16)(x1 - (float)h[1]);
  *hi = __builtin_bit_cast(unsigned, h);
  *lo = __builtin_bit_cast(unsigned, l);
}

template <int MT, int VW, int PAIR = 0>
__global__ __launch_bounds__(256) void wino_input_kernel(const WinoP p) {
  WINO_TL_BEGIN
  typedef typename VecT<VW>::T V;
  constexpr int N = MT + 2;
  static_assert(!PAIR || VW == 2, "pair operands: two channels per lane (one dword of hi, one of lo)");
  const int CV = p.C / VW;
  const long long per_tile = (long long)p.Z * CV;
  const long long total = (long long)p.B * p.TX * p.TY * per_tile;
  const V *in = reinterpret_cast<const V *>(p.in);
  V *Vw = reinterpret_cast<V *>(p.V);
  const float vscale = PAIR ? wino_pair_vscale(p.hdr) : 1.0f;
  const bool sat = PAIR ? wino_amax_bad(__uint_as_float(p.hdr[0])) : false;
  for (long long t = (long long)blockIdx.x * blockDim.x + threadIdx.x; t < total; t += (long long)gridDim.x * blockDim.x) {
    const long long zc = t % per_tile;
    long long q = t / per_tile;
    const int ty = (int)(q % p.TY);
    q /= p.TY;
    const int tx = (int)(q % p.TX);
    const int b = (int)(q / p.TX);
    const int x0 = MT * tx - p.px, y0 = MT * ty - p.py;
    V w[N][N];
#pragma unroll
    for (int j = 0; j < N; ++j) {
      const int y = y0 + j;
      V d[N];
#pragma unroll
      for (int i = 0; i < N; ++i) {
        const int x = x0 + i;
        const bool ok = (unsigned)x < (unsigned)p.X && (unsigned)y < (unsigned)p.Y;
        d[i] = ok ? in[(((long long)b * p.X + x) * p.Y + y) * per_tile + zc] : vzero((V *)nullptr);
      }
      V c[N];
      Wino1D<MT, V>::in(d, c);
#pragma unroll
      for (int i = 0; i < N; ++i) w[i][j] = c[i];
    }
#pragma unroll
    for (int i = 0; i < N; ++i) {
      V v[N];
      Wino1D<MT, V>::in(w[i], v);
      if constexpr (PAIR) {
        const int cv = (int)(zc % CV);
        const bool odd = cv & 1;
        const long long dw = 2 * (t - cv) + ((cv >> 3) << 4) + (cv & 6) + (odd ? 8 : 0);
        u32x2w *Vp = reinterpret_cast<u32x2w *>(reinterpret_cast<unsigned *>(p.V) + dw);
        const long long pstride = p.vs / 2;
#pragma unroll
        for (int j = 0; j < N; ++j) {
// ... 12 lines not shown
    }
  }
  WINO_TL_END(p)
}

__device__ __forceinline__ float wino_finish(const WinoP &p, float acc, float sc, float sf, float r) {
  float v = acc * sc + sf;
  if (p.res_mode && !p.res_after_act) v += r;
  if (p.relu) v = v > 0.f ? v : 0.f;
  if (p.res_mode && p.res_after_act) v += r;
  return v * p.post_scale;
}
__device__ __forceinline__ float4 wino_finish_v(const WinoP &p, float4 a, float4 sc, float4 sf, float4 r) {
  return make_float4(wino_finish(p, a.x, sc.x, sf.x, r.x), wino_finish(p, a.y, sc.y, sf.y, r.y), wino_finish(p, a.z, sc.z, sf.z, r.z),
                     wino_finish(p, a.w, sc.w, sf.w, r.w));
}
__device__ __forceinline__ float wino_finish_v(const WinoP &p, float a, float sc, float sf, float r) { return wino_finish(p, a, sc, sf, r); }
__device__ __forceinline__ float2 wino_finish_v(const WinoP &p, float2 a, float2 sc, float2 sf, float2 r) {
  return make_float2(wino_finish(p, a.x, sc.x, sf.x, r.x), wino_finish(p, a.y, sc.y, sf.y, r.y));
}

template <int MT, int VW>
__global__ __launch_bounds__(256) void wino_output_kernel(const WinoP p) {
  WINO_TL_BEGIN
  typedef typename VecT<VW>::T V;
  constexpr int N = MT + 2;
  const int CV = p.Co / VW;
  const long long per_tile = (long long)p.Zo * CV;
  const long long total = (long long)p.B * p.TX * p.TY * per_tile;
  const V *Mw = reinterpret_cast<const V *>(p.Mw);
  const V *res = reinterpret_cast<const V *>(p.res);
  V *out = reinterpret_cast<V *>(p.out);
  const float mscale = wino_mscale(p.hdr);
  float omax = 0.f;
  for (long long t = (long long)blockIdx.x * blockDim.x + threadIdx.x; t < total; t += (long long)gridDim.x * blockDim.x) {
    const long long zc = t % per_tile;
    const int cv = (int)(zc % CV);
    long long q = t / per_tile;
    const int ty = (int)(q % p.TY);
    q /= p.TY;
    const int tx = (int)(q % p.TX);
    const int b = (int)(q / p.TX);
    V r[MT][N];
#pragma unroll
    for (int j = 0; j < N; ++j) {
      V m[N];
#pragma unroll
      for (int i = 0; i < N; ++i) m[i] = Mw[(long long)(N * i + j) * (p.ms / VW) + t];
      V y[MT];
      Wino1D<MT, V>::out(m, y);
#pragma unroll
      for (int a = 0; a < MT; ++a) r[a][j] = y[a];
    }
    const V sc = mscale * (p.scale ? reinterpret_cast<const V *>(p.scale)[cv] : vone((V *)nullptr));
    const V sf = p.shift ? reinterpret_cast<const V *>(p.shift)[cv] : vzero((V *)nullptr);
#pragma unroll
    for (int a = 0; a < MT; ++a) {
      const int x = MT * tx + a;
      if (x >= p.Xo) continue;
      V yy[MT];
      Wino1D<MT, V>::out(r[a], yy);
#pragma unroll
      for (int e = 0; e < MT; ++e) {
        const int y = MT * ty + e;
        if (y >= p.Yo) continue;
        const long long o = (((long long)b * p.Xo + x) * p.Yo + y) * per_tile + zc;
        V rr = vzero((V *)nullptr);
        if (p.res_mode) rr = res[o];
        const V val = wino_finish_v(p, yy[e], sc, sf, rr);
        out[o] = val;
        if (p.pmax) omax = fmaxf(omax, vabsmax(val));
      }
    }
  }
  if (p.pmax) wino_block_max_store(omax, p.pmax);
  WINO_TL_END(p)
}

template <int MT> struct WinoAt;
template <> struct WinoAt<6> {
  static __device__ __forceinline__ float c(int e, int j) {
// ... 55 lines not shown
                                             const unsigned ps) {
    V nxt[8];
    if (J + 1 < 8) {
#pragma unroll
      for (int i = 0; i < 8; ++i) nxt[i] = BufIO<VW>::load(rm, vo, (unsigned)(8 * i + J + 1) * ps);
    }
    __builtin_amdgcn_sched_barrier(0);
    V y[6];
    Wino1D<6, V>::out(col, y);
#pragma unroll
    for (int a = 0; a < 6; ++a) wino6_acc_column<J>(acc[a], y[a]);
    __builtin_amdgcn_sched_barrier(0);
    Wino6Columns<J + 1, VW>::run(acc, nxt, rm, vo, ps);
  }
};
template <int VW> struct Wino6Columns<8, VW> {
  typedef typename VecT<VW>::T V;
  static __device__ __forceinline__ void run(V (&)[6][6], const V (&)[8], const __amdgpu_buffer_rsrc_t, const unsigned, const unsigned) {}
};

template <int VW, int WPE, int RPF = 0>
__global__ __launch_bounds__(256, WPE) void wino_output_buf_kernel(const WinoP p, const unsigned m_bytes, const unsigned out_bytes) {
  WINO_TL_BEGIN
  typedef typename VecT<VW>::T V;
  constexpr int MT = 6, N = 8, EB = VW * 4;
  const int CV = p.Co / VW;
  const long long per_tile = (long long)p.Zo * CV;
  const long long total = (long long)p.B * p.TX * p.TY * per_tile;
  const __amdgpu_buffer_rsrc_t rm = __builtin_amdgcn_make_buffer_rsrc((void *)p.Mw, 0, m_bytes, 0x00020000);
  const __amdgpu_buffer_rsrc_t ro = __builtin_amdgcn_make_buffer_rsrc((void *)p.out, 0, out_bytes, 0x00020000);
  const __amdgpu_buffer_rsrc_t rr = __builtin_amdgcn_make_buffer_rsrc((void *)(p.res ? p.res : p.out), 0, p.res ? out_bytes : 0u, 0x00020000);
  const unsigned ps = (unsigned)(p.ms * 4);
  const float mscale = wino_mscale(p.hdr);
  float omax = 0.f;
  for (long long t = (long long)blockIdx.x * blockDim.x + threadIdx.x; t < total; t += (long long)gridDim.x * blockDim.x) {
    const long long zc = t % per_tile;
    const int cv = (int)(zc % CV);
    long long q = t / per_tile;
    const int ty = (int)(q % p.TY);
    q /= p.TY;
    const int tx = (int)(q % p.TX);
    const int b = (int)(q / p.TX);
    const unsigned vo = (unsigned)(t * EB);
    const V sc = mscale * (p.scale ? reinterpret_cast<const V *>(p.scale)[cv] : vone((V *)nullptr));
    const V sf = p.shift ? reinterpret_cast<const V *>(p.shift)[cv] : vzero((V *)nullptr);
    const int xb = MT * tx, yb = MT * ty;
    const unsigned o00 = (unsigned)(((((long long)b * p.Xo + xb) * p.Yo + yb) * per_tile + zc) * EB);
    const unsigned row = (unsigned)(p.Yo * per_tile * EB), colb = (unsigned)(per_tile * EB);
    V rres[RPF ? MT : 1][RPF ? MT : 1];
    if constexpr (RPF) {
#pragma unroll
      for (int a = 0; a < MT; ++a)
#pragma unroll
        for (int e = 0; e < MT; ++e)
          rres[a][e] = BufIO<VW>::load(rr, (xb + a < p.Xo && yb + e < p.Yo) ? o00 : 0x80000000u, (unsigned)a * row + (unsigned)e * colb);
      __builtin_amdgcn_sched_barrier(0);
    }
    V acc[MT][MT];
#pragma unroll
    for (int a = 0; a < MT; ++a)
#pragma unroll
      for (int e = 0; e < MT; ++e) acc[a][e] = vzero((V *)nullptr);
    V col[N];
#pragma unroll
    for (int i = 0; i < N; ++i) col[i] = BufIO<VW>::load(rm, vo, (unsigned)(N * i) * ps);
    Wino6Columns<0, VW>::run(acc, col, rm, vo, ps);
#pragma unroll
    for (int a = 0; a < MT; ++a) {
#pragma unroll
      for (int e = 0; e < MT; ++e) {
        const unsigned vo_ae = (xb + a < p.Xo && yb + e < p.Yo) ? o00 : 0x80000000u;
        const unsigned so = (unsigned)a * row + (unsigned)e * colb;
        V rv;
        if constexpr (RPF) rv = rres[a][e];
        else rv = BufIO<VW>::load(rr, vo_ae, so);
        const V val = wino_finish_v(p, acc[a][e], sc, sf, rv);
// ... 59 lines not shown
int wino_dims(const ivx_conv_desc *d, int tile, WinoDims *w, const char *who) {
  IVX_REQUIRE(d, "%s: null descriptor", who);
  IVX_REQUIRE(tile == 2 || tile == 4 || tile == 6, "%s: tile must be 2, 4 or 6 (F(m x m, 3x3)), got %d", who, tile);
  IVX_REQUIRE(d->KD == 3 && d->KH == 3 && d->sd == 1 && d->sh == 1, "%s: needs a 3x3 kernel with stride 1 on the first two axes", who);
  IVX_REQUIRE(d->KW >= 1 && d->KW <= 8 && d->sw >= 1 && d->pd >= 0 && d->ph >= 0 && d->pw >= 0, "%s: bad z kernel / stride / padding", who);
  IVX_REQUIRE(d->B > 0 && d->D > 0 && d->H > 0 && d->W > 0, "%s: non-positive dims", who);
  IVX_REQUIRE(d->Cin > 0 && d->Cin % 4 == 0 && d->Cout > 0 && d->Cout % 4 == 0, "%s: Cin and Cout must be multiples of 4", who);
  IVX_REQUIRE(d->in_dtype == IVX_F32 && d->out_dtype == IVX_F32, "%s: fp32 only", who);
  IVX_REQUIRE(d->wino_operands == IVX_F32 || (d->wino_operands == IVX_F16_PAIR && tile >= 4 && d->Cin % 16 == 0 &&
                                               (d->wgt_layout == 0 || d->Cin % 32 == 0)),
              "%s: wino_operands is IVX_F32 or IVX_F16_PAIR (tile 4 / 6, Cin %% 16 == 0; wgt_layout 1: Cin %% 32 == 0)", who);
  IVX_REQUIRE(d->out_mode == 0 && (d->res_mode == 0 || d->res_mode == 1), "%s: out_mode 0 and res_mode 0/1 only", who);
  IVX_REQUIRE(d->wgt_layout == 0 || (d->wgt_layout == 1 && d->Cin % 32 == 0), "%s: wgt_layout 1 needs Cin %% 32 == 0", who);
  int32_t Xo, Yo, Zo;
  if (ivx_conv_out_dims(d, &Xo, &Yo, &Zo) != IVX_OK) return IVX_ERR_INVALID_ARG;
  w->Xo = Xo; w->Yo = Yo; w->Zo = Zo;
  w->TX = (Xo + tile - 1) / tile; w->TY = (Yo + tile - 1) / tile;
  w->n2 = (tile + 2) * (tile + 2);
  w->v_elems = (int64_t)d->B * w->TX * w->TY * d->W * d->Cin;
  w->m_elems = (int64_t)d->B * w->TX * w->TY * Zo * d->Cout;
  w->v_stride = w->v_elems;
  w->m_stride = w->m_elems;
  return IVX_OK;
}

ivx_conv_desc wino_group_desc(const ivx_conv_desc *d, const WinoDims &w) {
  ivx_conv_desc g = *d;
  g.D = w.TX; g.H = w.TY;
  g.KD = 1; g.KH = 1; g.pd = 0; g.ph = 0; g.sd = 1; g.sh = 1;
  g.relu = 0; g.res_mode = 0; g.res_h = 0; g.res_w = 0; g.res_after_act = 0; g.post_scale = 1.0f;
  return g;
}

unsigned wino_blocks(int64_t items) {
  const int64_t b = (items + 255) / 256;
  return (unsigned)(b < 1 ? 1 : (b > (1 << 20) ? (1 << 20) : b));
}

}

extern "C" int ivx_conv_winograd_set_variant(int32_t output_variant, int32_t input_variant) {
  g_wino_out_variant = output_variant;
  g_wino_in_variant = input_variant;
  return IVX_OK;
}

extern "C" int ivx_conv_winograd_supported(const ivx_conv_desc *d, int32_t tile) {
  WinoDims w;
  if (wino_dims(d, tile, &w, "ivx_conv_winograd_supported") != IVX_OK) return 0;
  if (w.v_stride * 4 >= (1LL << 31) || w.m_stride >= (1LL << 31) - 512 * (int64_t)d->Cout) return 0;
  if ((int64_t)d->Cout * d->KW * d->Cin * 4 >= (1LL << 31)) return 0;
  return 1;
}

extern "C" int64_t ivx_conv_winograd_weight_elems(const ivx_conv_desc *d, int32_t tile) {
  WinoDims w;
  if (wino_dims(d, tile, &w, "ivx_conv_winograd_weight_elems") != IVX_OK) return -1;
  return (int64_t)(w.n2 + (d->wino_operands == IVX_F16_PAIR ? 1 : 0)) * d->Cout * d->KW * d->Cin;
}

extern "C" int ivx_conv_winograd_weights(const ivx_conv_desc *d, int32_t tile, const float *wgt, float *u, ivx_stream_t stream) {
  WinoDims w;
  int rc = wino_dims(d, tile, &w, "ivx_conv_winograd_weights");
  if (rc != IVX_OK) return rc;
  IVX_REQUIRE(wgt && u, "ivx_conv_winograd_weights: null argument");
  const int64_t total = (int64_t)d->Cout * d->KW * d->Cin;
// ... 24 lines not shown
  return ivx_align_up(w.n2 * w.v_stride * 4, 256) + ivx_align_up(w.n2 * w.m_stride * 4, 256) + 256;
}

namespace {
#ifdef IVX_CONV_TIMELINE
unsigned long long *g_wino_timeline = nullptr;
#endif
int wino_setup(const ivx_conv_desc *d, int tile, const void *in, const float *scale, const float *shift, const void *res, void *out,
               void *workspace, int64_t workspace_bytes, WinoDims *w, WinoP *p, const char *who) {
  int rc = wino_dims(d, tile, w, who);
  if (rc != IVX_OK) return rc;
  IVX_REQUIRE(workspace, "%s: null workspace", who);
  if (!ivx_conv_winograd_supported(d, tile)) {
    ivx_set_error("%s: one transformed plane must stay below 2 GiB (use ivx_conv_fwd)", who);
    return IVX_ERR_UNSUPPORTED;
  }
  const int64_t need = ivx_conv_winograd_workspace_bytes(d, tile);
  if (workspace_bytes < need) {
    ivx_set_error("%s: workspace too small (%lld < %lld); size it with ivx_conv_winograd_workspace_bytes", who,
                  (long long)workspace_bytes, (long long)need);
    return IVX_ERR_WORKSPACE;
  }
  p->in = (const float *)in; p->scale = scale; p->shift = shift; p->res = d->res_mode ? (const float *)res : nullptr;
  p->out = (float *)out;
  p->V = (float *)workspace;
  p->Mw = (float *)((char *)workspace + ivx_align_up(w->n2 * w->v_stride * 4, 256));
  p->vs = w->v_stride; p->ms = w->m_stride;
  p->B = d->B; p->X = d->D; p->Y = d->H; p->Z = d->W; p->C = d->Cin;
  p->Xo = w->Xo; p->Yo = w->Yo; p->Zo = w->Zo; p->Co = d->Cout;
  p->TX = w->TX; p->TY = w->TY; p->px = d->pd; p->py = d->ph;
  p->relu = d->relu; p->res_mode = d->res_mode; p->res_after_act = d->res_after_act;
  p->post_scale = d->post_scale == 0.f ? 1.0f : d->post_scale;
  p->pmax = nullptr;
#ifdef IVX_CONV_TIMELINE
  p->tl = g_wino_timeline;
#endif
  p->hdr = d->wino_operands == IVX_F16_PAIR
               ? (const unsigned *)((char *)workspace + ivx_align_up(w->n2 * w->v_stride * 4, 256) + ivx_align_up(w->n2 * w->m_stride * 4, 256))
               : nullptr;
  return IVX_OK;
}
}

static int wino_input_impl(const ivx_conv_desc *d, int32_t tile, const void *in, void *workspace, int64_t workspace_bytes,
                           const float *partials, int32_t n_partials, ivx_stream_t stream) {
  WinoDims w;
  WinoP p;
  float dummy;
  IVX_REQUIRE(in, "ivx_conv_winograd_input: null argument");
  int rc = wino_setup(d, tile, in, nullptr, nullptr, &dummy, &dummy, workspace, workspace_bytes, &w, &p, "ivx_conv_winograd_input");
  if (rc != IVX_OK) return rc;
  if (d->wino_operands == IVX_F16_PAIR) {
    static const bool one_wg = !(getenv("IVX_WINO_AMAX_ONE_WG") && atoi(getenv("IVX_WINO_AMAX_ONE_WG")) == 0);
    const bool write_form = partials && n_partials <= 65536 && one_wg;
    if (!write_form && hipMemsetAsync((void *)p.hdr, 0, 4, (hipStream_t)stream) != hipSuccess) {
      ivx_set_error("ivx_conv_winograd_input: hipMemsetAsync failed");
      return IVX_ERR_HIP;
    }
    if (write_form) {
      hipLaunchKernelGGL(wino_amax_partials_write_kernel, dim3(1), dim3(1024), 0, (hipStream_t)stream, partials, n_partials, (unsigned *)p.hdr);
    } else if (partials) {
      const int pb = (n_partials + 255) / 256;
      hipLaunchKernelGGL(wino_amax_partials_kernel, dim3((unsigned)(pb > 64 ? 64 : pb)), dim3(256), 0, (hipStream_t)stream, partials, n_partials,
                         (unsigned *)p.hdr);
    } else {
      const size_t n4 = (size_t)d->B * d->D * d->H * d->W * d->Cin / 4;
      const size_t ab = (n4 + 1023) / 1024;
      hipLaunchKernelGGL(wino_amax_kernel, dim3((unsigned)(ab > 1536 ? 1536 : (ab < 1 ? 1 : ab))), dim3(256), 0, (hipStream_t)stream,
                         (const wf32x4 *)in, n4, (unsigned *)p.hdr);
    }
    if (tile == 4)
      hipLaunchKernelGGL((wino_input_kernel<4, 2, 1>), dim3(wino_blocks(w.v_elems / 2)), dim3(256), 0, (hipStream_t)stream, p);
    else
      hipLaunchKernelGGL((wino_input_kernel<6, 2, 1>), dim3(wino_blocks(w.v_elems / 2)), dim3(256), 0, (hipStream_t)stream, p);
  } else if (tile == 2)
    hipLaunchKernelGGL((wino_input_kernel<2, 4>), dim3(wino_blocks(w.v_elems / 4)), dim3(256), 0, (hipStream_t)stream, p);
  else if (tile == 4)
    hipLaunchKernelGGL((wino_input_kernel<4, 2>), dim3(wino_blocks(w.v_elems / 2)), dim3(256), 0, (hipStream_t)stream, p);
  else if (g_wino_in_variant == 1)
    hipLaunchKernelGGL((wino_input_kernel<6, 1>), dim3(wino_blocks(w.v_elems)), dim3(256), 0, (hipStream_t)stream, p);
  else
    hipLaunchKernelGGL((wino_input_kernel<6, 2>), dim3(wino_blocks(w.v_elems / 2)), dim3(256), 0, (hipStream_t)stream, p);
  IVX_CHECK_LAUNCH("ivx_conv_winograd_input");
  return IVX_OK;
}

extern "C" int ivx_conv_winograd_input(const ivx_conv_desc *d, int32_t tile, const void *in, void *workspace, int64_t workspace_bytes,
                                       ivx_stream_t stream) {
  return wino_input_impl(d, tile, in, workspace, workspace_bytes, nullptr, 0, stream);
}

extern "C" int ivx_conv_winograd_input_amax(const ivx_conv_desc *d, int32_t tile, const void *in, void *workspace, int64_t workspace_bytes,
                                            const float *partials, int32_t n_partials, ivx_stream_t stream) {
  IVX_REQUIRE(!partials || n_partials > 0, "ivx_conv_winograd_input_amax: partials without a count");
  return wino_input_impl(d, tile, in, workspace, workspace_bytes, partials, n_partials, stream);
}

extern "C" int ivx_conv_winograd_gemm(const ivx_conv_desc *d, int32_t tile, const float *u, void *workspace, int64_t workspace_bytes,
                                      ivx_stream_t stream) {
  WinoDims w;
  WinoP p;
  float dummy;
  IVX_REQUIRE(u, "ivx_conv_winograd_gemm: null argument");
  int rc = wino_setup(d, tile, &dummy, nullptr, nullptr, &dummy, &dummy, workspace, workspace_bytes, &w, &p, "ivx_conv_winograd_gemm");
  if (rc != IVX_OK) return rc;
  ivx_conv_desc g = wino_group_desc(d, w);
  const long long el = d->wino_operands == IVX_F16_PAIR ? 2 : 1;
  g.in_dtype = d->wino_operands;
  const unsigned *us = p.hdr ? reinterpret_cast<const unsigned *>(u + (int64_t)w.n2 * d->Cout * d->KW * d->Cin + 1) : nullptr;
  rc = ivx_conv_grouped_launch(&g, w.n2, p.V, el * w.v_stride, u, el * d->Cout * d->KW * d->Cin, p.Mw, w.m_stride, (hipStream_t)stream, us,
                               p.hdr ? const_cast<unsigned *>(p.hdr) + 1 : nullptr);
  if (rc != IVX_OK) return rc;
  IVX_CHECK_LAUNCH("ivx_conv_winograd_gemm");
  return IVX_OK;
}

extern "C" int ivx_conv_winograd_fused_supported(const ivx_conv_desc *d, int32_t tile) {
  WinoDims w;
  if (tile != 4 || !d || d->wino_operands != IVX_F16_PAIR || d->KW != 3 || d->sw != 1 || d->pw != 1 || d->wgt_layout != 1 || d->Cin % 32 || d->Cout % 4)
    return 0;
  if (!ivx_conv_winograd_supported(d, tile) || wino_dims(d, tile, &w, "ivx_conv_winograd_fused_supported") != IVX_OK) return 0;
  if ((int64_t)w.n2 * w.v_stride * 4 >= (1LL << 31) || (int64_t)w.n2 * d->Cout * d->KW * d->Cin * 4 >= (1LL << 31)) return 0;
  return 1;
}

extern "C" int32_t ivx_conv_winograd_fused_blocks(const ivx_conv_desc *d, int32_t tile) {
  WinoDims w;
  if (!ivx_conv_winograd_fused_supported(d, tile) || wino_dims(d, tile, &w, "ivx_conv_winograd_fused_blocks") != IVX_OK) return -1;
  return ivx_conv_fold4_blocks((long long)d->B * w.TX * w.TY * w.Zo, d->Cout);
}

extern "C" int ivx_conv_winograd_gemm_output_amax(const ivx_conv_desc *d, int32_t tile, const float *u, const float *scale, const float *shift,
                                                  const void *res, void *out, void *workspace, int64_t workspace_bytes, float *partials,
                                                  ivx_stream_t stream) {
  WinoDims w;
  WinoP p;
  float dummy;
  IVX_REQUIRE(u && out, "ivx_conv_winograd_gemm_output: null argument");
  IVX_REQUIRE(!d || d->res_mode == 0 || res, "ivx_conv_winograd_gemm_output: res_mode set but res is NULL");
  if (!ivx_conv_winograd_fused_supported(d, tile)) {
    ivx_set_error("ivx_conv_winograd_gemm_output: the fused form takes F(4x4,3x3) on IVX_F16_PAIR operands, a 3-tap z kernel with stride 1 and padding 1, "
                  "wgt_layout 1, Cin %% 32 == 0, and all 36 planes of V below 2 GiB (ivx_conv_winograd_fused_supported)");
    return IVX_ERR_UNSUPPORTED;
  }
  int rc = wino_setup(d, tile, &dummy, scale, shift, res, out, workspace, workspace_bytes, &w, &p, "ivx_conv_winograd_gemm_output");
  if (rc != IVX_OK) return rc;
  ivx_conv_desc g = wino_group_desc(d, w);
// ... 9 lines not shown
  if (fold_waves == 2 && d->Cout % 8 == 0)
    rc = ivx_conv_launch_fold4w(reinterpret_cast<const _Float16 *>(p.V), 2 * w.v_stride, reinterpret_cast<const _Float16 *>(u), 2LL * d->Cout * d->KW * d->Cin,
                                d->B * w.TX * w.TY * w.Zo, 2 * d->Cin, d->Cout, w.Zo, f, (hipStream_t)stream);
  else
    rc = ivx_conv_grouped_fold4(&g, w.n2, p.V, 2 * w.v_stride, u, 2LL * d->Cout * d->KW * d->Cin, &f, (hipStream_t)stream);
  if (rc != IVX_OK) return rc;
  IVX_CHECK_LAUNCH("ivx_conv_winograd_gemm_output");
  return IVX_OK;
}

namespace {
int wino_output_variant(const ivx_conv_desc *d, const WinoDims &w, bool with_partials) {
  const bool buf_ok = (int64_t)w.n2 * w.m_stride * 4 < (1LL << 32) && (int64_t)d->B * w.Xo * w.Yo * w.Zo * d->Cout * 4 < (1LL << 31);
  int v = (g_wino_out_variant >= 0 && !with_partials) ? g_wino_out_variant : (d->res_mode ? 4 : 1);
  if (v >= 2 && !buf_ok) v = 0;
  if (v >= 4 && !d->res_mode) v = v == 4 ? 2 : 3;
  return v;
}
unsigned wino_output_grid(const ivx_conv_desc *d, int tile, const WinoDims &w, bool with_partials) {
  if (tile == 2) return wino_blocks(w.m_elems / 4);
  if (tile == 4) return wino_blocks(w.m_elems / 2);
  const int v = wino_output_variant(d, w, with_partials);
  return (v == 2 || v == 0 || v == 4) ? wino_blocks(w.m_elems / 2) : wino_blocks(w.m_elems);
}
}

extern "C" int32_t ivx_conv_winograd_output_blocks(const ivx_conv_desc *d, int32_t tile) {
  WinoDims w;
  if (wino_dims(d, tile, &w, "ivx_conv_winograd_output_blocks") != IVX_OK) return -1;
  return (int32_t)wino_output_grid(d, tile, w, true);
}

static int wino_output_impl(const ivx_conv_desc *d, int32_t tile, const float *scale, const float *shift, const void *res, void *out,
                            void *workspace, int64_t workspace_bytes, float *partials, ivx_stream_t stream) {
  WinoDims w;
  WinoP p;
  float dummy;
  IVX_REQUIRE(out, "ivx_conv_winograd_output: null argument");
  IVX_REQUIRE(!d || d->res_mode == 0 || res, "ivx_conv_winograd_output: res_mode set but res is NULL");
  int rc = wino_setup(d, tile, &dummy, scale, shift, res, out, workspace, workspace_bytes, &w, &p, "ivx_conv_winograd_output");
  if (rc != IVX_OK) return rc;
  p.pmax = partials;
  if (tile == 2)
    hipLaunchKernelGGL((wino_output_kernel<2, 4>), dim3(wino_blocks(w.m_elems / 4)), dim3(256), 0, (hipStream_t)stream, p);
  else if (tile == 4)
    hipLaunchKernelGGL((wino_output_kernel<4, 2>), dim3(wino_blocks(w.m_elems / 2)), dim3(256), 0, (hipStream_t)stream, p);
  else {
    const int v = wino_output_variant(d, w, partials != nullptr);
    const unsigned mb = (unsigned)((int64_t)w.n2 * w.m_stride * 4), ob = (unsigned)((int64_t)d->B * w.Xo * w.Yo * w.Zo * d->Cout * 4);
    if (v == 2)
      hipLaunchKernelGGL((wino_output_buf_kernel<2, 3>), dim3(wino_blocks(w.m_elems / 2)), dim3(256), 0, (hipStream_t)stream, p, mb, ob);
    else if (v == 3)
      hipLaunchKernelGGL((wino_output_buf_kernel<1, 5>), dim3(wino_blocks(w.m_elems)), dim3(256), 0, (hipStream_t)stream, p, mb, ob);
    else if (v == 4)
      hipLaunchKernelGGL((wino_output_buf_kernel<2, 2, 1>), dim3(wino_blocks(w.m_elems / 2)), dim3(256), 0, (hipStream_t)stream, p, mb, ob);
    else if (v == 5)
      hipLaunchKernelGGL((wino_output_buf_kernel<1, 4, 1>), dim3(wino_blocks(w.m_elems)), dim3(256), 0, (hipStream_t)stream, p, mb, ob);
    else if (v == 1)
      hipLaunchKernelGGL((wino_output_kernel<6, 1>), dim3(wino_blocks(w.m_elems)), dim3(256), 0, (hipStream_t)stream, p);
    else
      hipLaunchKernelGGL((wino_output_kernel<6, 2>), dim3(wino_blocks(w.m_elems / 2)), dim3(256), 0, (hipStream_t)stream, p);
  }
  IVX_CHECK_LAUNCH("ivx_conv_winograd_output");
  return IVX_OK;
}

extern "C" int ivx_conv_winograd_output(const ivx_conv_desc *d, int32_t tile, const float *scale, const float *shift, const void *res,
                                        void *out, void *workspace, int64_t workspace_bytes, ivx_stream_t stream) {
  return wino_output_impl(d, tile, scale, shift, res, out, workspace, workspace_bytes, nullptr, stream);
}

extern "C" int ivx_conv_winograd_output_amax(const ivx_conv_desc *d, int32_t tile, const float *scale, const float *shift, const void *res,
                                             void *out, void *workspace, int64_t workspace_bytes, float *partials, ivx_stream_t stream) {
  return wino_output_impl(d, tile, scale, shift, res, out, workspace, workspace_bytes, partials, stream);
}

extern "C" int ivx_conv_winograd_fwd(const ivx_conv_desc *d, int32_t tile, const void *in, const float *u, const float *scale,
                                     const float *shift, const void *res, void *out, void *workspace, int64_t workspace_bytes,
                                     ivx_stream_t stream) {
  int rc = ivx_conv_winograd_input(d, tile, in, workspace, workspace_bytes, stream);
  if (rc != IVX_OK) return rc;
  rc = ivx_conv_winograd_gemm(d, tile, u, workspace, workspace_bytes, stream);
  if (rc != IVX_OK) return rc;
  return ivx_conv_winograd_output(d, tile, scale, shift, res, out, workspace, workspace_bytes, stream);
}

#ifdef IVX_CONV_TIMELINE
extern "C" int ivx_wino_set_timeline(void *buf) { g_wino_timeline = (unsigned long long *)buf; return 0; }
#endif
```

imvoxelnet_amd/ops.py:

```python
import ctypes as C

import torch

from . import _lib
from ._lib import ConvDesc, AnchorHeadDesc, check


def _stream():
    return C.c_void_p(torch.cuda.current_stream().cuda_stream)


FP8 = torch.float8_e4m3fn
_DT = {torch.float32: 0, torch.bfloat16: 1, FP8: 2}


def _chk(t, name, dtype=torch.float32):
    if not isinstance(t, torch.Tensor):
        raise TypeError(f'{name} must be a torch.Tensor')
    if not t.is_cuda:
        raise RuntimeError(f'{name} must be a device (HIP) tensor; the MI355X path has no CPU fallback')
    if t.dtype != dtype:
        raise TypeError(f'{name} must be {dtype}, got {t.dtype}')
    if not t.is_contiguous():
        raise ValueError(f'{name} must be contiguous')
# ... 154 lines not shown

def _wino_desc(B, D, H, W, Cin, Cout, kw, stride_w, padding, relu, wgt_layout, res_mode=0, res_after_act=False, post_scale=1.0, operands=0):
    return ConvDesc(B, D, H, W, Cin, Cout, 3, 3, kw, 1, 1, stride_w, padding[0], padding[1], padding[2], int(bool(relu)),
                    int(res_mode), 0, 0, int(wgt_layout), 0, int(bool(res_after_act)), float(post_scale), 0, 0, 1.0, int(operands))


def conv_winograd_supported(x_shape, Cout, kernel, stride, padding, tile=2, operands=0):
    if kernel[0] != 3 or kernel[1] != 3 or stride[0] != 1 or stride[1] != 1 or x_shape[4] % 4 or Cout % 4 or tile not in (2, 4, 6):
        return False
    B, D, H, W, Cin = x_shape
    d = _wino_desc(B, D, H, W, Cin, Cout, kernel[2], stride[2], padding, False, 0, operands=operands)
    return bool(_lib.lib().ivx_conv_winograd_supported(C.byref(d), tile))


def conv_winograd_weights(wgt, wgt_layout, tile=2, operands=0):
    _chk(wgt, 'wgt')
    Cout, kd, kh, kw, Cin = wgt.shape
    if kd != 3 or kh != 3:
        raise ValueError('Winograd F(m x m, 3x3) needs a 3x3 kernel on the first two axes')
    d = _wino_desc(1, 4, 4, max(kw, 1), Cin, Cout, kw, 1, (1, 1, kw // 2), False, wgt_layout, operands=operands)
    L = _lib.lib()
    n = L.ivx_conv_winograd_weight_elems(C.byref(d), tile)
    if n < 0:
        check(-1, 'ivx_conv_winograd_weight_elems')
    u = torch.empty(((tile + 2) ** 2 + (1 if operands else 0), Cout, kw * Cin), device=wgt.device, dtype=torch.float32)
    assert u.numel() == n
    check(L.ivx_conv_winograd_weights(C.byref(d), tile, _ptr(wgt), _ptr(u), _stream()), 'ivx_conv_winograd_weights')
    return u


winograd_trace = None


def conv_winograd_fwd(x, u, scale=None, shift=None, kw=3, stride_w=1, padding=(1, 1, 1), relu=False, res=None, out=None,
                      wgt_layout=0, res_after_act=False, post_scale=1.0, operands=0, amax_in=None, want_amax=False, fused=False):
    _chk(x, 'x')
    _chk(u, 'u')
    B, D, H, W, Cin = x.shape
    Cout = u.shape[1]
    tile = {16: 2, 36: 4, 64: 6}.get(u.shape[0] - (1 if operands else 0))
    if tile is None or tuple(u.shape[1:]) != (Cout, kw * Cin):
        raise ValueError(f'transformed filters {tuple(u.shape)} do not match kw {kw} / Cin {Cin}')
    d = _wino_desc(B, D, H, W, Cin, Cout, kw, stride_w, padding, relu, wgt_layout, 1 if res is not None else 0, res_after_act,
                   post_scale, operands)
    do, ho, wo = C.c_int32(), C.c_int32(), C.c_int32()
    L = _lib.lib()
    check(L.ivx_conv_out_dims(C.byref(d), C.byref(do), C.byref(ho), C.byref(wo)), 'ivx_conv_out_dims')
    oshape = (B, do.value, ho.value, wo.value, Cout)
    if res is not None:
        _chk(res, 'res')
        if tuple(res.shape) != oshape:
            raise ValueError(f'residual shape {tuple(res.shape)} != output shape')
    for t, n in ((scale, 'scale'), (shift, 'shift')):
        if t is not None:
            _chk(t, n)
            if t.numel() != Cout:
                raise ValueError(f'{n} must have {Cout} elements')
    if out is None:
        out = torch.empty(oshape, device=x.device, dtype=torch.float32)
    else:
        _chk(out, 'out')
    wsb = L.ivx_conv_winograd_workspace_bytes(C.byref(d), tile)
    if wsb < 0:
        check(-1, 'ivx_conv_winograd_workspace_bytes')
    ws = torch.empty((wsb,), device=x.device, dtype=torch.uint8)
    if fused:
        if not L.ivx_conv_winograd_fused_supported(C.byref(d), tile):
            raise ValueError('this layer does not take the fused GEMM + output form (ivx_conv_winograd_fused_supported)')
        part = None
        if want_amax:
            part = torch.empty((L.ivx_conv_winograd_fused_blocks(C.byref(d), tile),), device=x.device, dtype=torch.float32)
        if amax_in is not None:
            _chk(amax_in, 'amax_in')
        check(L.ivx_conv_winograd_input_amax(C.byref(d), tile, _ptr(x), _ptr(ws), wsb, _ptr(amax_in), 0 if amax_in is None else amax_in.numel(),
                                             _stream()), 'ivx_conv_winograd_input_amax')
        check(L.ivx_conv_winograd_gemm_output_amax(C.byref(d), tile, _ptr(u), _ptr(scale), _ptr(shift), _ptr(res), _ptr(out), _ptr(ws), wsb, _ptr(part),
                                                   _stream()), 'ivx_conv_winograd_gemm_output_amax')
        return (out, part) if want_amax else out
    if amax_in is not None or want_amax:
        part = None
        if want_amax:
            nb = L.ivx_conv_winograd_output_blocks(C.byref(d), tile)
            if nb < 0:
                check(-1, 'ivx_conv_winograd_output_blocks')
            part = torch.empty((nb,), device=x.device, dtype=torch.float32)
        if amax_in is not None:
            _chk(amax_in, 'amax_in')
        check(L.ivx_conv_winograd_input_amax(C.byref(d), tile, _ptr(x), _ptr(ws), wsb, _ptr(amax_in), 0 if amax_in is None else amax_in.numel(),
                                             _stream()), 'ivx_conv_winograd_input_amax')
        check(L.ivx_conv_winograd_gemm(C.byref(d), tile, _ptr(u), _ptr(ws), wsb, _stream()), 'ivx_conv_winograd_gemm')
        check(L.ivx_conv_winograd_output_amax(C.byref(d), tile, _ptr(scale), _ptr(shift), _ptr(res), _ptr(out), _ptr(ws), wsb, _ptr(part),
                                              _stream()), 'ivx_conv_winograd_output_amax')
        return (out, part) if want_amax else out
    if winograd_trace is None:
        check(L.ivx_conv_winograd_fwd(C.byref(d), tile, _ptr(x), _ptr(u), _ptr(scale), _ptr(shift), _ptr(res), _ptr(out), _ptr(ws),
                                      wsb, _stream()), 'ivx_conv_winograd_fwd')
        return out
    ev = [torch.cuda.Event(enable_timing=True) for _ in range(4)]
    ev[0].record()
    check(L.ivx_conv_winograd_input(C.byref(d), tile, _ptr(x), _ptr(ws), wsb, _stream()), 'ivx_conv_winograd_input')
    ev[1].record()
    check(L.ivx_conv_winograd_gemm(C.byref(d), tile, _ptr(u), _ptr(ws), wsb, _stream()), 'ivx_conv_winograd_gemm')
    ev[2].record()
    check(L.ivx_conv_winograd_output(C.byref(d), tile, _ptr(scale), _ptr(shift), _ptr(res), _ptr(out), _ptr(ws), wsb, _stream()),
          'ivx_conv_winograd_output')
    ev[3].record()
    tiles = B * ((oshape[1] + tile - 1) // tile) * ((oshape[2] + tile - 1) // tile)
    winograd_trace.append(('input', ev[0], ev[1], 0.0))
    frac = float(L.ivx_conv_winograd_issued_fraction(C.byref(d)))
    winograd_trace.append(('gemm', ev[1], ev[2], (3.0 if operands else 1.0) * frac * 2.0 * (tile + 2) ** 2 * tiles * oshape[3] * Cout * kw * Cin))
# ... 758 lines not shown
```

include/imvoxel.h:

```cpp
#ifndef IMVOXEL_H_
#define IMVOXEL_H_

#include <stdint.h>

#ifdef __cplusplus
extern "C" {
#endif

#define IVX_OK 0
#define IVX_ERR_INVALID_ARG (-1)
#define IVX_ERR_HIP (-2)
#define IVX_ERR_UNSUPPORTED (-3)
#define IVX_ERR_WORKSPACE (-4)

typedef void *ivx_stream_t;

int ivx_version(void);
const char *ivx_last_error(void);

#define IVX_F32 0
#define IVX_BF16 1
#define IVX_FP8 2
#define IVX_BF16_PAIR 3
#define IVX_F16_PAIR 4
// ... 92 lines not shown
                           ivx_stream_t stream);
int ivx_conv_winograd_output(const ivx_conv_desc *d, int32_t tile, const float *scale, const float *shift, const void *res,
                             void *out, void *workspace, int64_t workspace_bytes, ivx_stream_t stream);
int ivx_conv_winograd_fwd(const ivx_conv_desc *d, int32_t tile, const void *in, const float *u, const float *scale,
                          const float *shift, const void *res, void *out, void *workspace, int64_t workspace_bytes,
                          ivx_stream_t stream);
typedef struct ivx_conv_route_opts {
  int32_t winograd;
  int32_t winograd_tile;
  int32_t wino_operands;
  int32_t split;
  int64_t winograd_min_pos;
  int32_t winograd_2d_min_ch;
} ivx_conv_route_opts;
typedef struct ivx_conv_route {
  int32_t form;
  int32_t tile;
  int32_t wino_candidate, split_candidate;
  int32_t split_fits;
  int32_t prefers_winograd;
  ivx_conv_desc run;
} ivx_conv_route_out;
int ivx_conv_route(const ivx_conv_desc *d, int32_t cin_real, const ivx_conv_route_opts *o, ivx_conv_route_out *r);
int32_t ivx_conv_winograd_output_blocks(const ivx_conv_desc *d, int32_t tile);
int ivx_conv_winograd_output_amax(const ivx_conv_desc *d, int32_t tile, const float *scale, const float *shift, const void *res, void *out,
                                  void *workspace, int64_t workspace_bytes, float *partials, ivx_stream_t stream);
int ivx_conv_winograd_input_amax(const ivx_conv_desc *d, int32_t tile, const void *in, void *workspace, int64_t workspace_bytes,
                                 const float *partials, int32_t n_partials, ivx_stream_t stream);
int ivx_conv_winograd_fused_supported(const ivx_conv_desc *d, int32_t tile);
int32_t ivx_conv_winograd_fused_blocks(const ivx_conv_desc *d, int32_t tile);
int ivx_conv_winograd_gemm_output_amax(const ivx_conv_desc *d, int32_t tile, const float *u, const float *scale, const float *shift,
                                       const void *res, void *out, void *workspace, int64_t workspace_bytes, float *partials,
                                       ivx_stream_t stream);


int ivx_dcn_im2col_fwd(const float *x, const float *offset_mask, int32_t B, int32_t H, int32_t W, int32_t C, int32_t kh,
                       int32_t kw, int32_t stride, int32_t pad, int32_t dil, int32_t om_channels, float *col,
                       ivx_stream_t stream);
int ivx_dcn_im2col_fwd_pair(const void *x, const float *x_scale, const float *offset_mask, int32_t B, int32_t H, int32_t W, int32_t C,
                            int32_t kh, int32_t kw, int32_t stride, int32_t pad, int32_t dil, int32_t om_channels, void *col,
                            float *col_scale, uint32_t *col_amax, ivx_stream_t stream);
int ivx_dcn_im2col_fwd_bf16(const void *x, const float *offset_mask, int32_t B, int32_t H, int32_t W, int32_t C, int32_t kh,
                            int32_t kw, int32_t stride, int32_t pad, int32_t dil, int32_t om_channels, void *col,
                            ivx_stream_t stream);

int ivx_maxpool2d_fwd(const float *in, int32_t B, int32_t H, int32_t W, int32_t C, int32_t k,
                      int32_t s, int32_t p, float *out, ivx_stream_t stream);
int ivx_maxpool2d_fwd_bf16(const void *in, int32_t B, int32_t H, int32_t W, int32_t C, int32_t k,
                           int32_t s, int32_t p, void *out, ivx_stream_t stream);
int ivx_maxpool2d_fwd_fp8(const void *in, int32_t B, int32_t H, int32_t W, int32_t C, int32_t k, int32_t s, int32_t p,
                          void *out, ivx_stream_t stream);

int ivx_upsample_trilinear2x_fwd(const float *in, int32_t B, int32_t D, int32_t H, int32_t W, int32_t C, float *out,
                                 ivx_stream_t stream);

int ivx_nchw_to_nhwc(const float *in, int32_t B, int32_t C, int64_t S, int32_t Cpad, float *out,
                     ivx_stream_t stream);
int ivx_image_s2d_bf16(const float *img, int32_t B, int32_t H, int32_t W, void *out, ivx_stream_t stream);
int ivx_nhwc_to_nchw(const float *in, int32_t B, int64_t S, int32_t C, float *out, ivx_stream_t stream);

#define IVX_IMAGE_PREP_MAX_DIM 32768
typedef struct ivx_image_prep_desc {
  int32_t src_h, src_w;
  int32_t src_row_bytes;
  int32_t dst_h, dst_w;
  int32_t pad_h, pad_w;
// ... 266 lines not shown
```

Before: 262.6 images/s.

## Skip background Winograd tiles in the 3-D neck chain via device-side row compaction

Adds a background plan built on the device from the back-projection validity mask. For each layer of the chained 3x3x3 Winograd neck convolutions it computes which 6x6 output tiles can be affected by visible voxels, growing the region layer by layer. The input transform, grouped GEMM and output transform then process only those compacted tiles. The halo and z-blocked GEMM kernels now read their row count from device memory, so the host needs no synchronisation. The path is on by default and adds planning kernels and workspace, and it relies on the background handling in the output stage being exact for tiles that are skipped.

```diff
diff --git a/imvoxelnet_amd/_lib.py b/imvoxelnet_amd/_lib.py
--- a/imvoxelnet_amd/_lib.py
+++ b/imvoxelnet_amd/_lib.py
@@ -122,6 +122,8 @@
 
 
 EXPORTS = ['ivx_model_plan_info', 'ivx_model_plan_step', 'ivx_model_plan_tensor', 'ivx_bottleneck_proj_supported', 'ivx_bottleneck_proj_pack', 'ivx_bottleneck_proj_fwd_pio', 'ivx_anchor_head_decode', 'ivx_fcos3d_head_decode', 'ivx_nms_rotated_bev', 'ivx_nms_aligned3d', 'ivx_bottleneck_supported', 'ivx_bottleneck_fwd_pio', 'ivx_amax_f32', 'ivx_stem_pool_filter_bytes', 'ivx_stem_pool_pack_filters', 'ivx_stem_pool_out_dims', 'ivx_stem_pool_fwd_pair', 'ivx_conv_winograd_set_variant', 'ivx_ubench_mfma', 'ivx_ubench_copy', 'ivx_version', 'ivx_last_error', 'ivx_conv_out_dims', 'ivx_conv_fwd', 'ivx_conv_fwd_naive', 'ivx_conv_set_tile_override', 'ivx_conv_set_epilogue_mode', 'ivx_conv_set_plan_mode', 'ivx_topk_set_mode', 'ivx_conv_workspace_bytes', 'ivx_conv_fwd_ws', 'ivx_conv_set_halo_mode', 'ivx_bf16_pair_split', 'ivx_f16_pair_split', 'ivx_conv_pair_supported', 'ivx_bf16_pair_pack_filters', 'ivx_conv_route', 'ivx_conv_pio_workspace_bytes', 'ivx_conv_fwd_pio', 'ivx_conv_fwd_pio_naive', 'ivx_pair_pack_filters', 'ivx_nchw_to_nhwc_amax', 'ivx_maxpool2d_fwd_pair', 'ivx_f16_pair_merge', 'ivx_model_calibrate_fp8', 'ivx_model_calibrate_fp8_ex', 'ivx_amax_bf16', 'ivx_conv_winograd_output_blocks', 'ivx_conv_winograd_issued_fraction', 'ivx_conv_winograd_output_amax', 'ivx_conv_winograd_input_amax', 'ivx_conv_winograd_fused_supported', 'ivx_conv_winograd_fused_blocks', 'ivx_conv_winograd_gemm_output_amax',
+           'ivx_conv_winograd_bg_supported', 'ivx_conv_winograd_bg_bytes', 'ivx_conv_winograd_bg_layer_offset', 'ivx_conv_winograd_bg_plan',
+           'ivx_conv_winograd_input_bg', 'ivx_conv_winograd_gemm_bg', 'ivx_conv_winograd_output_bg',
            'ivx_conv_winograd_supported', 'ivx_conv_winograd_weight_elems', 'ivx_conv_winograd_weights', 'ivx_conv_winograd_workspace_bytes',
            'ivx_conv_winograd_input', 'ivx_conv_winograd_gemm', 'ivx_conv_winograd_output', 'ivx_conv_winograd_fwd',
            'ivx_maxpool2d_fwd', 'ivx_maxpool2d_fwd_bf16', 'ivx_maxpool2d_fwd_fp8', 'ivx_global_avgpool_fwd', 'ivx_global_avgpool_fwd_bf16', 'ivx_upsample_trilinear2x_fwd', 'ivx_dcn_im2col_fwd', 'ivx_dcn_im2col_fwd_bf16', 'ivx_dcn_im2col_fwd_pair', 'ivx_nchw_to_nhwc', 'ivx_image_s2d_bf16', 'ivx_nhwc_to_nchw', 'ivx_backproject_mean_fwd', 'ivx_backproject_mean_fwd_amax', 'ivx_backproject_amax_blocks', 'ivx_backproject_mean_fwd_bf16', 'ivx_upsample_trilinear2x_fwd_bf16', 'ivx_backproject_sum_fwd', 'ivx_volume_normalize_fwd',
@@ -166,6 +168,15 @@
     L.ivx_conv_winograd_fused_blocks.argtypes = [C.POINTER(ConvDesc), i32]
     L.ivx_conv_winograd_fused_blocks.restype = i32
     L.ivx_conv_winograd_gemm_output_amax.argtypes = [C.POINTER(ConvDesc), i32, vp, vp, vp, vp, vp, vp, i64, vp, vp]
+    L.ivx_conv_winograd_bg_supported.argtypes = [C.POINTER(ConvDesc), i32]
+    L.ivx_conv_winograd_bg_bytes.argtypes = [C.POINTER(ConvDesc), i32]
+    L.ivx_conv_winograd_bg_bytes.restype = i64
+    L.ivx_conv_winograd_bg_layer_offset.argtypes = [C.POINTER(ConvDesc), i32]
+    L.ivx_conv_winograd_bg_layer_offset.restype = i64
+    L.ivx_conv_winograd_bg_plan.argtypes = [C.POINTER(ConvDesc), vp, i32, C.POINTER(i32), vp, i64, vp]
+    L.ivx_conv_winograd_input_bg.argtypes = [C.POINTER(ConvDesc), i32, vp, vp, i64, vp, i32, vp, vp]
+    L.ivx_conv_winograd_gemm_bg.argtypes = [C.POINTER(ConvDesc), i32, vp, vp, i64, vp, vp]
+    L.ivx_conv_winograd_output_bg.argtypes = [C.POINTER(ConvDesc), i32, vp, vp, vp, vp, vp, i64, vp, vp, vp]
     L.ivx_bf16_pair_split.argtypes = [vp, i64, vp, vp]
     L.ivx_f16_pair_split.argtypes = [vp, i64, f32, vp, vp]
     L.ivx_conv_pair_supported.argtypes = [C.POINTER(ConvDesc)]
diff --git a/imvoxelnet_amd/csrc/conv_igemm.hip b/imvoxelnet_amd/csrc/conv_igemm.hip
--- a/imvoxelnet_amd/csrc/conv_igemm.hip
+++ b/imvoxelnet_amd/csrc/conv_igemm.hip
@@ -56,6 +56,7 @@
   float wbound, sbound;
   const unsigned *cp_src;
   unsigned *cp_dst;
+  const int *m_dev;
   int stagger_ticks, stagger_shift, stagger_first;
 #ifdef IVX_CONV_TIMELINE
   unsigned long long *tl;
@@ -1288,7 +1289,7 @@
 #ifdef IVX_CONV_TIMELINE
   p->tl = g_timeline;
 #endif
-  p->cp_src = nullptr; p->cp_dst = nullptr;
+  p->cp_src = nullptr; p->cp_dst = nullptr; p->m_dev = nullptr;
   p->pio = 0; p->in_scale_p = nullptr; p->out_pair = 0; p->res_pair = 0; p->res_scale_p = nullptr; p->out_scale_p = nullptr;
   p->amax_in = p->amax_res = nullptr; p->amax_out = nullptr; p->wbound = 0.f; p->sbound = 0.f;
   if (io) {
@@ -1640,18 +1641,21 @@
   static_assert(sizeof(smem) >= (size_t)NT / 64 * 4096, "4 KB of staging LDS per wave for the transposed epilogue");
   const int tid = threadIdx.x, lane = tid & 63, wid = tid >> 6;
   const int wr = wid / WC, wc = wid % WC;
+  const int M = p.m_dev ? *p.m_dev : p.M;
+  const int q_total = p.m_dev ? ((M + BMO - 1) / BMO + 7) >> 3 : p.q_total;
   int mt, nt;
   {
     const int Nt = (p.Cout + BN - 1) / BN;
     const int xcd = blockIdx.x & 7, idx = blockIdx.x >> 3;
     const int lt = idx / Nt;
     nt = idx - lt * Nt;
-    mt = xcd * p.q_total + lt;
-  }
-  if (mt * BMO >= p.M) return;
+    mt = xcd * q_total + lt;
+    if (p.cp_dst && blockIdx.x == 0 && blockIdx.z == 0 && tid == 0) *p.cp_dst = *p.cp_src;
+    if (lt >= q_total) return;
+  }
+  if (mt * BMO >= M) return;
   const int m0 = mt * BMO, n0 = nt * BN;
   const size_t gz = blockIdx.z;
-  if (p.cp_dst && blockIdx.x == 0 && blockIdx.z == 0 && tid == 0) *p.cp_dst = *p.cp_src;
 #ifdef IVX_CONV_TIMELINE
   const unsigned long long tl0 = __builtin_amdgcn_s_memrealtime();
   unsigned long long tl1 = 0, tl2 = 0;
@@ -1672,7 +1676,7 @@
     const int li = j < APASS ? lr + RP * j : BM + (lane >> 2);
     const int row = SW * m0 - 1 + (DI ? (li < BM ? 2 * li : 2 * (li - BM) + 1) : li);
     const bool zr = ZR && !TAIL && li == ZROW;
-    a_base[j] = (row >= 0 && row < SW * p.M && (j < APASS || (lane >> 2) < 2) && !zr) ? ((unsigned)row * (unsigned)p.Cin + cc * EPC) * (unsigned)sizeof(T) : OOB;
+    a_base[j] = (row >= 0 && row < SW * M && (j < APASS || (lane >> 2) < 2) && !zr) ? ((unsigned)row * (unsigned)p.Cin + cc * EPC) * (unsigned)sizeof(T) : OOB;
   }
   unsigned b_base[BPASS];
 #pragma unroll
@@ -1804,7 +1808,7 @@
   } else {
     float *stage = reinterpret_cast<float *>(smem) + wid_u * 1024;
     float *outp = p.out + gz * (size_t)p.g_out;
-    const int mlim = (m0 + BMO < p.M) ? m0 + BMO : p.M;
+    const int mlim = (m0 + BMO < M) ? m0 + BMO : M;
     const int col_l = lane & 31, hh = lane >> 5, rrow = lane >> 3, c4 = (lane & 7) * 4;
 #pragma unroll
     for (int j = 0; j < TN; ++j) {
@@ -1861,23 +1865,26 @@
   const int tid = threadIdx.x, lane = tid & 63, wid = tid >> 6;
   const int wid_u = __builtin_amdgcn_readfirstlane(wid);
   const int cg = wid_u / (ZH * WN), zh = (wid_u / WN) % ZH, nb = wid_u % WN;
+  const int M = p.m_dev ? *p.m_dev : p.M;
+  const int q_total = p.m_dev ? ((M + CT * Z - 1) / (CT * Z) + 7) >> 3 : p.q_total;
   int mt, nt;
   {
     const int Nt = (p.Cout + BN - 1) / BN;
     const int xcd = blockIdx.x & 7, idx = blockIdx.x >> 3;
     const int lt = idx / Nt;
     nt = idx - lt * Nt;
-    mt = xcd * p.q_total + lt;
+    mt = xcd * q_total + lt;
+    if (p.cp_dst && blockIdx.x == 0 && blockIdx.z == 0 && tid == 0) *p.cp_dst = *p.cp_src;
+    if (lt >= q_total) return;
   }
   const int c0 = mt * CT, n0 = nt * BN;
   const int m0 = c0 * Z;
-  if (m0 >= p.M) return;
+  if (m0 >= M) return;
 #ifdef IVX_CONV_TIMELINE
   const unsigned long long tl0 = __builtin_amdgcn_s_memrealtime();
   unsigned long long tl1 = 0, tl2 = 0;
 #endif
   const size_t gz = blockIdx.z;
-  if (p.cp_dst && blockIdx.x == 0 && blockIdx.z == 0 && tid == 0) *p.cp_dst = *p.cp_src;
   const __amdgpu_buffer_rsrc_t rs_in =
       __builtin_amdgcn_make_buffer_rsrc((void *)((const char *)p.in + gz * (size_t)p.g_in * sizeof(T)), 0, in_bytes, 0x00020000);
   const __amdgpu_buffer_rsrc_t rs_w =
@@ -1892,7 +1899,7 @@
     const int li = lr + RP * j;
     const int z = li / CT, c = li - z * CT;
     const int row = (c0 + c) * ZI + z;
-    a_base[j] = (li < AR && row < SW * p.M) ? ((unsigned)row * (unsigned)p.Cin + cc * EPC) * (unsigned)sizeof(T) : OOB;
+    a_base[j] = (li < AR && row < SW * M) ? ((unsigned)row * (unsigned)p.Cin + cc * EPC) * (unsigned)sizeof(T) : OOB;
   }
 #pragma unroll
   for (int j = 0; j < BPASS; ++j) {
@@ -1982,7 +1989,7 @@
     for (int q = 0; q < 4; ++q) {
       const f32x4 v = *reinterpret_cast<const f32x4 *>(stage + (rrow + 8 * q) * 32 + c4);
       const int m = m0 + (cg * 32 + rrow + 8 * q) * Z + z0 + zo;
-      if (m < p.M && nok) *reinterpret_cast<f32x4 *>(outp + (size_t)m * p.Cout + nbc) = v;
+      if (m < M && nok) *reinterpret_cast<f32x4 *>(outp + (size_t)m * p.Cout + nbc) = v;
     }
   }
 #ifdef IVX_CONV_TIMELINE
@@ -2534,8 +2541,30 @@
   return 7.0f / 9.0f;
 }
 
+static int grouped_halo_cfg(const ConvParams &p, const ivx_conv_desc *d, int groups) {
+  if (p.in_pair == 2 && p.kmode == 1 && d->KD == 1 && d->KH == 1 && d->KW == 3 && d->sw == 2 && d->pw == 1 && p.W == 2 * p.Wo && p.Cin % 64 == 0 &&
+      ((g_halo_mode >= 21 && g_halo_mode < 30) || (g_halo_mode >= 40 && g_halo_mode < 50) || g_halo_mode >= 70 || (g_halo_mode < 0 && g_tile_override == 0))) {
+    return g_halo_mode >= 21 ? g_halo_mode : 42;
+  }
+  if (p.in_pair == 2 && p.kmode == 1 && d->KD == 1 && d->KH == 1 && d->KW == 3 && d->sw == 1 && d->pw == 1 && p.Cin % 64 == 0 &&
+      ((g_halo_mode > 0 && g_halo_mode < 21) || (g_halo_mode >= 30 && g_halo_mode < 40) || (g_halo_mode >= 50 && g_halo_mode < 70) ||
+       (g_halo_mode < 0 && g_tile_override == 0))) {
+    static const int halo_small = getenv("IVX_HALO_SMALL") ? atoi(getenv("IVX_HALO_SMALL")) : 1;
+    const bool few = halo_small && p.Cout > 64 && !zblk_rule(p) && (long long)((p.M + 252) / 253) * ((p.Cout + 127) / 128) * groups < 512;
+    return g_halo_mode > 0 ? g_halo_mode : ((p.Cout <= 64 || few) ? 30 : (zblk_rule(p) ? 50 : 33));
+  }
+  return 0;
+}
+
+int ivx_conv_grouped_rows_dev_ok(const ivx_conv_desc *d, int groups) {
+  ConvParams p;
+  float dummy;
+  if (!d || fill_params(d, &dummy, &dummy, nullptr, nullptr, nullptr, &dummy, &p) != IVX_OK || !dma_applicable(p)) return 0;
+  return grouped_halo_cfg(p, d, groups) != 0;
+}
+
 int ivx_conv_grouped_launch(const ivx_conv_desc *d, int groups, const float *in, long long g_in, const float *wgt, long long g_w,
-                            float *out, long long g_out, hipStream_t st, const unsigned *cp_src, unsigned *cp_dst) {
+                            float *out, long long g_out, hipStream_t st, const unsigned *cp_src, unsigned *cp_dst, const int *m_dev) {
   ConvParams p;
   int rc = fill_params(d, in, wgt, nullptr, nullptr, nullptr, out, &p);
   if (rc != IVX_OK) return rc;
@@ -2556,17 +2585,11 @@
     p.cp_src = cp_src; p.cp_dst = cp_dst;
   }
   p.groups = groups; p.g_in = g_in; p.g_w = g_w; p.g_out = g_out;
-  if (p.in_pair == 2 && p.kmode == 1 && d->KD == 1 && d->KH == 1 && d->KW == 3 && d->sw == 2 && d->pw == 1 && p.W == 2 * p.Wo && p.Cin % 64 == 0 &&
-      ((g_halo_mode >= 21 && g_halo_mode < 30) || (g_halo_mode >= 40 && g_halo_mode < 50) || g_halo_mode >= 70 || (g_halo_mode < 0 && g_tile_override == 0))) {
-    return ivx_conv_launch_halo(p, g_halo_mode >= 21 ? g_halo_mode : 42, st);
-  }
-  if (p.in_pair == 2 && p.kmode == 1 && d->KD == 1 && d->KH == 1 && d->KW == 3 && d->sw == 1 && d->pw == 1 && p.Cin % 64 == 0 &&
-      ((g_halo_mode > 0 && g_halo_mode < 21) || (g_halo_mode >= 30 && g_halo_mode < 40) || (g_halo_mode >= 50 && g_halo_mode < 70) ||
-       (g_halo_mode < 0 && g_tile_override == 0))) {
-    static const int halo_small = getenv("IVX_HALO_SMALL") ? atoi(getenv("IVX_HALO_SMALL")) : 1;
-    const bool few = halo_small && p.Cout > 64 && !zblk_rule(p) && (long long)((p.M + 252) / 253) * ((p.Cout + 127) / 128) * groups < 512;
-    const int cfg = g_halo_mode > 0 ? g_halo_mode : ((p.Cout <= 64 || few) ? 30 : (zblk_rule(p) ? 50 : 33));
-    return ivx_conv_launch_halo(p, cfg, st);
+  p.m_dev = m_dev;
+  if (const int halo_cfg = grouped_halo_cfg(p, d, groups)) return ivx_conv_launch_halo(p, halo_cfg, st);
+  if (m_dev) {
+    ivx_set_error("ivx_conv_grouped_launch: only the z-halo and z-blocked kernels take a device-side row count");
+    return IVX_ERR_UNSUPPORTED;
   }
   ConvPlan pl = {g_tile_override, 1, 1, 0, 0, 0, 0};
   if (pl.cfg == 0 && p.in_pair) {
diff --git a/imvoxelnet_amd/csrc/model.cpp b/imvoxelnet_amd/csrc/model.cpp
--- a/imvoxelnet_amd/csrc/model.cpp
+++ b/imvoxelnet_amd/csrc/model.cpp
@@ -14,6 +14,21 @@
 #include "../../include/imvoxel_lab.h"
 
 void ivx_set_error(const char *fmt, ...);
+
+extern "C" {
+__attribute__((weak)) int ivx_conv_winograd_bg_supported(const ivx_conv_desc *d, int32_t tile);
+__attribute__((weak)) int64_t ivx_conv_winograd_bg_bytes(const ivx_conv_desc *d, int32_t n_layers);
+__attribute__((weak)) int64_t ivx_conv_winograd_bg_layer_offset(const ivx_conv_desc *d, int32_t layer);
+__attribute__((weak)) int ivx_conv_winograd_bg_plan(const ivx_conv_desc *d, const uint8_t *valid, int32_t n_layers, const int32_t *out_slices, void *block,
+                                                    int64_t block_bytes, ivx_stream_t stream);
+__attribute__((weak)) int ivx_conv_winograd_input_bg(const ivx_conv_desc *d, int32_t tile, const void *in, void *workspace, int64_t workspace_bytes,
+                                                     const float *partials, int32_t n_partials, const int32_t *bg, ivx_stream_t stream);
+__attribute__((weak)) int ivx_conv_winograd_gemm_bg(const ivx_conv_desc *d, int32_t tile, const float *u, void *workspace, int64_t workspace_bytes,
+                                                    const int32_t *bg, ivx_stream_t stream);
+__attribute__((weak)) int ivx_conv_winograd_output_bg(const ivx_conv_desc *d, int32_t tile, const float *scale, const float *shift, const void *res,
+                                                      void *out, void *workspace, int64_t workspace_bytes, float *partials, const int32_t *bg,
+                                                      ivx_stream_t stream);
+}
 
 #define M_REQUIRE(cond, ...)        \
   do {                              \
@@ -158,6 +173,7 @@
   int bound_layer = -1;
   int fuse = 0, fuse_out = -1;
   int side = 0, join = 0;
+  int64_t bg = -1;
 };
 
 struct Plan {
@@ -173,6 +189,9 @@
   int64_t ws2_off = 0, ws2_bytes = 0;
   int n_sides = 0;
   int s0 = 0, s1 = 0;
+  int bg_first = -1, bg_layers = 0;
+  int64_t bg_off = -1, bg_bytes = 0;
+  int32_t bg_zo[9] = {0, 0, 0, 0, 0, 0, 0, 0, 0};
 };
 
 }
@@ -206,7 +225,11 @@
   bool trace_on = false;
   bool trace_skip = false;
   int trace_level = 2;
-  struct TraceRec { int step, stage, is3d; double flops, bytes; hipEvent_t e0, e1; std::string name; };
+  struct TraceRec {
+    int step, stage, is3d; double flops, bytes; hipEvent_t e0, e1; std::string name;
+    const int32_t *rows_dev = nullptr;
+    double rows_dense = 0.0;
+  };
   std::vector<TraceRec> trace;
   std::vector<hipEvent_t> event_pool;
   size_t events_used = 0;
@@ -1157,6 +1180,37 @@
       break;
     }
   }
+  const bool bg_on = !(getenv("IVX_NECK_BACKGROUND") && atoi(getenv("IVX_NECK_BACKGROUND")) == 0);
+  if (bg_on && ivx_conv_winograd_bg_plan && ivx_conv_winograd_bg_supported && m->lift_step >= r.s0 && m->lift_step < r.s1 && c.storage == IVX_F32) {
+    std::vector<int> chain_t = {m->steps[m->lift_step].out};
+    std::vector<int> chain_s;
+    for (int i = m->lift_step + 1; i < r.s1 && (int)chain_s.size() < 9; ++i) {
+      const Step &s = m->steps[i];
+      const PlanStep &ps = pl->ps[i];
+      if (s.kind != ST_CONV || s.in != chain_t.back() || ps.tile != 6 || !ivx_conv_winograd_bg_supported(&ps.d, ps.tile)) break;
+      if (s.res >= 0 && (s.res_mode != 1 || std::find(chain_t.begin(), chain_t.end(), s.res) == chain_t.end())) break;
+      if (!chain_s.empty()) {
+        const ivx_conv_desc &d0 = pl->ps[chain_s[0]].d;
+        if (ps.d.B != d0.B || ps.d.D != d0.D || ps.d.H != d0.H) break;
+      }
+      int32_t xo, yo, zo;
+      M_TRY(ivx_conv_out_dims(&ps.d, &xo, &yo, &zo));
+      pl->bg_zo[chain_s.size()] = zo;
+      chain_s.push_back(i);
+      chain_t.push_back(s.out);
+    }
+    if (!chain_s.empty()) {
+      const ivx_conv_desc &d0 = pl->ps[chain_s[0]].d;
+      pl->bg_first = chain_s[0];
+      pl->bg_layers = (int)chain_s.size();
+      pl->bg_bytes = ivx_conv_winograd_bg_bytes(&d0, pl->bg_layers);
+      M_REQUIRE(pl->bg_bytes > 0, "background plan: %s", ivx_last_error());
+      top = align256(top);
+      pl->bg_off = top;
+      top += align256(pl->bg_bytes);
+      for (size_t l = 0; l < chain_s.size(); ++l) pl->ps[chain_s[l]].bg = pl->bg_off + ivx_conv_winograd_bg_layer_offset(&d0, (int32_t)l);
+    }
+  }
   if (n_slots > 0) {
     top = align256(top);
     pl->scal_off = top;
@@ -1287,6 +1341,25 @@
   auto scalep = [&](int t) -> float * { uint32_t *q = slotp(t); return q ? (float *)(q + IVX_AMAX_SLOTS) : nullptr; };
   if (pl.scal_bytes > 0 && r.s0 <= m->trunk0 && r.s1 > m->trunk0)
     M_HIP(hipMemsetAsync(base + pl.scal_off, 0, (size_t)pl.scal_bytes, st), "hipMemsetAsync (amax slots)");
+  auto wino_input = [&](const PlanStep &ps, const void *in) -> int {
+    const float *part = ps.amax_in >= 0 ? (const float *)(base + ps.amax_in) : nullptr;
+    if (ps.bg >= 0) return ivx_conv_winograd_input_bg(&ps.d, ps.tile, in, ws, pl.ws_bytes, part, ps.amax_in_n, (const int32_t *)(base + ps.bg), st);
+    return ivx_conv_winograd_input_amax(&ps.d, ps.tile, in, ws, pl.ws_bytes, part, ps.amax_in_n, st);
+  };
+  auto wino_gemm = [&](const PlanStep &ps, const ConvLayer &L) -> int {
+    const float *u = L.u.at(ps.tile * 8 + ps.d.wino_operands);
+    if (ps.bg >= 0) return ivx_conv_winograd_gemm_bg(&ps.d, ps.tile, u, ws, pl.ws_bytes, (const int32_t *)(base + ps.bg), st);
+    return ivx_conv_winograd_gemm(&ps.d, ps.tile, u, ws, pl.ws_bytes, st);
+  };
+  auto wino_output = [&](const PlanStep &ps, const ConvLayer &L, const void *res, void *out) -> int {
+    float *part = ps.amax_out >= 0 ? (float *)(base + ps.amax_out) : nullptr;
+    if (ps.bg >= 0) return ivx_conv_winograd_output_bg(&ps.d, ps.tile, L.scale, L.shift, res, out, ws, pl.ws_bytes, part, (const int32_t *)(base + ps.bg), st);
+    return ivx_conv_winograd_output_amax(&ps.d, ps.tile, L.scale, L.shift, res, out, ws, pl.ws_bytes, part, st);
+  };
+  auto bg_plan = [&](const Step &lift) -> int {
+    if (pl.bg_first < 0) return IVX_OK;
+    return ivx_conv_winograd_bg_plan(&pl.ps[pl.bg_first].d, (const uint8_t *)ptr(lift.out2), pl.bg_layers, pl.bg_zo, base + pl.bg_off, pl.bg_bytes, st);
+  };
   const bool span2d = m->trace_on && m->trace_level == 1 && m->cfg.with_trunk;
   std::vector<char> forked((size_t)std::max(pl.n_sides, 1), 0);
   double span_flops = 0.0, span_bytes = 0.0;
@@ -1455,16 +1528,18 @@
           M_TRY(ivx_conv_out_dims(&ps.d, &zo_d, &zo_h, &zo));
           const double vb = 4.0 * n * n * tiles * ps.d.W * ps.d.Cin, mb = 4.0 * n * n * tiles * zo * ps.d.Cout;
           M_TRY(trace_begin(m, i, 1, is3d, 0.0, 4.0 * in.elems() + vb, L.name, st));
-          M_TRY(ivx_conv_winograd_input_amax(&ps.d, ps.tile, ptr(s.in), ws, pl.ws_bytes, ps.amax_in >= 0 ? (const float *)(base + ps.amax_in) : nullptr,
-                                             ps.amax_in_n, st));
+          M_TRY(wino_input(ps, ptr(s.in)));
           M_TRY(trace_end(m, st));
           M_TRY(trace_begin(m, i, 2, is3d, (ps.d.wino_operands ? 3.0 : 1.0) * ivx_conv_winograd_issued_fraction(&ps.d) * 2.0 * n * n * tiles * zo * ps.d.Cout * ps.d.KW * ps.d.Cin,
                             vb + mb, L.name, st));
-          M_TRY(ivx_conv_winograd_gemm(&ps.d, ps.tile, L.u.at(ps.tile * 8 + ps.d.wino_operands), ws, pl.ws_bytes, st));
+          if (ps.bg >= 0 && m->trace_on && !m->trace_skip) {
+            m->trace.back().rows_dev = (const int32_t *)(base + ps.bg) + 1;
+            m->trace.back().rows_dense = (double)tiles * zo;
+          }
+          M_TRY(wino_gemm(ps, L));
           M_TRY(trace_end(m, st));
           M_TRY(trace_begin(m, i, 3, is3d, 0.0, mb + 4.0 * o.elems() * (res ? 2 : 1), L.name, st));
-          M_TRY(ivx_conv_winograd_output_amax(&ps.d, ps.tile, L.scale, L.shift, res, ptr(s.out), ws, pl.ws_bytes,
-                                              ps.amax_out >= 0 ? (float *)(base + ps.amax_out) : nullptr, st));
+          M_TRY(wino_output(ps, L, res, ptr(s.out)));
           M_TRY(trace_end(m, st));
           break;
         }
@@ -1480,11 +1555,9 @@
           io.wbound = L.wbound; io.sbound = L.sbound;
           M_TRY(ivx_conv_fwd_pio(&ps.d, &io, ptr(s.in), L.wpair, L.scale_p, L.shift, res, ptr(s.out), cws, cws_bytes, cst));
         } else if (ps.tile) {
-          M_TRY(ivx_conv_winograd_input_amax(&ps.d, ps.tile, ptr(s.in), ws, pl.ws_bytes, ps.amax_in >= 0 ? (const float *)(base + ps.amax_in) : nullptr,
-                                             ps.amax_in_n, st));
-          M_TRY(ivx_conv_winograd_gemm(&ps.d, ps.tile, L.u.at(ps.tile * 8 + ps.d.wino_operands), ws, pl.ws_bytes, st));
-          M_TRY(ivx_conv_winograd_output_amax(&ps.d, ps.tile, L.scale, L.shift, res, ptr(s.out), ws, pl.ws_bytes,
-                                              ps.amax_out >= 0 ? (float *)(base + ps.amax_out) : nullptr, st));
+          M_TRY(wino_input(ps, ptr(s.in)));
+          M_TRY(wino_gemm(ps, L));
+          M_TRY(wino_output(ps, L, res, ptr(s.out)));
         } else if (m->fp8_on && L.fp8_eff) {
           M_TRY(ivx_conv_fwd_ws(&ps.d, ptr(s.in), L.fp8_eff >= 2 ? L.wq : L.w, L.scale_q, L.shift_q, res, ptr(s.out), cws, cws_bytes, cst));
         } else if (ps.split) {
@@ -1512,6 +1585,7 @@
           ld.sampling = m->cfg.sampling;
           M_TRY(ivx_backproject_fwd_ex(&ld, ptr(s.in), bd.proj, bd.new_origin, bd.crop, ptr(s.out), nullptr, nullptr, (uint8_t *)ptr(s.out2), st));
           M_TRY(trace_end(m, st));
+          M_TRY(bg_plan(s));
           break;
         }
         if (m->cfg.storage == IVX_BF16) {
@@ -1528,6 +1602,7 @@
                                             o.D, o.H, o.W, (float *)ptr(s.out), (uint8_t *)ptr(s.out2),
                                             pl.ps[i].amax_out >= 0 ? (float *)(base + pl.ps[i].amax_out) : nullptr, st));
         M_TRY(trace_end(m, st));
+        M_TRY(bg_plan(s));
         break;
       }
       case ST_DCN_COL: {
@@ -2180,7 +2255,13 @@
   float ms = 0.f, start = 0.f;
   M_HIP(hipEventElapsedTime(&ms, r.e0, r.e1), "hipEventElapsedTime (synchronise the stream first)");
   M_HIP(hipEventElapsedTime(&start, m->trace[0].e0, r.e0), "hipEventElapsedTime");
-  rec->step = r.step; rec->stage = r.stage; rec->is3d = r.is3d; rec->ms = ms; rec->start_ms = start; rec->flops = r.flops; rec->bytes = r.bytes;
+  double flops = r.flops;
+  if (r.rows_dev && r.rows_dense > 0.0) {
+    int32_t rows = 0;
+    M_HIP(hipMemcpy(&rows, r.rows_dev, sizeof(rows), hipMemcpyDeviceToHost), "hipMemcpy (GEMM row count)");
+    flops *= (double)rows / r.rows_dense;
+  }
+  rec->step = r.step; rec->stage = r.stage; rec->is3d = r.is3d; rec->ms = ms; rec->start_ms = start; rec->flops = flops; rec->bytes = r.bytes;
   snprintf(rec->name, sizeof(rec->name), "%s", r.name.c_str());
   return IVX_OK;
 }
diff --git a/imvoxelnet_amd/csrc/winograd.hip b/imvoxelnet_amd/csrc/winograd.hip
--- a/imvoxelnet_amd/csrc/winograd.hip
+++ b/imvoxelnet_amd/csrc/winograd.hip
@@ -4,12 +4,15 @@
                            hipStream_t st);
 
 int ivx_conv_grouped_launch(const ivx_conv_desc *d, int groups, const float *in, long long g_in, const float *wgt, long long g_w,
-                            float *out, long long g_out, hipStream_t st, const unsigned *cp_src, unsigned *cp_dst);
+                            float *out, long long g_out, hipStream_t st, const unsigned *cp_src, unsigned *cp_dst, const int *m_dev);
+int ivx_conv_grouped_rows_dev_ok(const ivx_conv_desc *d, int groups);
 int ivx_conv_grouped_fold4(const ivx_conv_desc *d, int groups, const float *in, long long g_in, const float *wgt, long long g_w, const IvxWinoFold *f,
                            hipStream_t st);
 int ivx_conv_fold4_blocks(long long M, int Cout);
 
 namespace {
+
+constexpr int WINO_BG_HDR = 4;
 
 struct WinoP {
   const float *in, *scale, *shift, *res;
@@ -24,6 +27,7 @@
   float post_scale;
   float *pmax;
   const unsigned *hdr;
+  const int *bg;
 #ifdef IVX_CONV_TIMELINE
   unsigned long long *tl;
 #endif
@@ -260,7 +264,8 @@
   static_assert(!PAIR || VW == 2, "pair operands: two channels per lane (one dword of hi, one of lo)");
   const int CV = p.C / VW;
   const long long per_tile = (long long)p.Z * CV;
-  const long long total = (long long)p.B * p.TX * p.TY * per_tile;
+  const int *lst = p.bg ? p.bg + WINO_BG_HDR : nullptr;
+  const long long total = (lst ? (long long)p.bg[0] : (long long)p.B * p.TX * p.TY) * per_tile;
   const V *in = reinterpret_cast<const V *>(p.in);
   V *Vw = reinterpret_cast<V *>(p.V);
   const float vscale = PAIR ? wino_pair_vscale(p.hdr) : 1.0f;
@@ -268,6 +273,7 @@
   for (long long t = (long long)blockIdx.x * blockDim.x + threadIdx.x; t < total; t += (long long)gridDim.x * blockDim.x) {
     const long long zc = t % per_tile;
     long long q = t / per_tile;
+    if (lst) q = lst[q];
     const int ty = (int)(q % p.TY);
     q /= p.TY;
     const int tx = (int)(q % p.TX);
@@ -346,11 +352,13 @@
   const V *res = reinterpret_cast<const V *>(p.res);
   V *out = reinterpret_cast<V *>(p.out);
   const float mscale = wino_mscale(p.hdr);
+  const int *src = p.bg ? p.bg + WINO_BG_HDR + p.B * p.TX * p.TY : nullptr;
   float omax = 0.f;
   for (long long t = (long long)blockIdx.x * blockDim.x + threadIdx.x; t < total; t += (long long)gridDim.x * blockDim.x) {
     const long long zc = t % per_tile;
     const int cv = (int)(zc % CV);
     long long q = t / per_tile;
+    const long long tm = src ? (long long)src[q] * per_tile + zc : t;
     const int ty = (int)(q % p.TY);
     q /= p.TY;
     const int tx = (int)(q % p.TX);
@@ -360,7 +368,7 @@
     for (int j = 0; j < N; ++j) {
       V m[N];
 #pragma unroll
-      for (int i = 0; i < N; ++i) m[i] = Mw[(long long)(N * i + j) * (p.ms / VW) + t];
+      for (int i = 0; i < N; ++i) m[i] = Mw[(long long)(N * i + j) * (p.ms / VW) + tm];
       V y[MT];
       Wino1D<MT, V>::out(m, y);
 #pragma unroll
@@ -482,16 +490,17 @@
   const __amdgpu_buffer_rsrc_t rr = __builtin_amdgcn_make_buffer_rsrc((void *)(p.res ? p.res : p.out), 0, p.res ? out_bytes : 0u, 0x00020000);
   const unsigned ps = (unsigned)(p.ms * 4);
   const float mscale = wino_mscale(p.hdr);
+  const int *src = p.bg ? p.bg + WINO_BG_HDR + p.B * p.TX * p.TY : nullptr;
   float omax = 0.f;
   for (long long t = (long long)blockIdx.x * blockDim.x + threadIdx.x; t < total; t += (long long)gridDim.x * blockDim.x) {
     const long long zc = t % per_tile;
     const int cv = (int)(zc % CV);
     long long q = t / per_tile;
+    const unsigned vo = (unsigned)((src ? (long long)src[q] * per_tile + zc : t) * EB);
     const int ty = (int)(q % p.TY);
     q /= p.TY;
     const int tx = (int)(q % p.TX);
     const int b = (int)(q / p.TX);
-    const unsigned vo = (unsigned)(t * EB);
     const V sc = mscale * (p.scale ? reinterpret_cast<const V *>(p.scale)[cv] : vone((V *)nullptr));
     const V sf = p.shift ? reinterpret_cast<const V *>(p.shift)[cv] : vzero((V *)nullptr);
     const int xb = MT * tx, yb = MT * ty;
@@ -617,6 +626,121 @@
   return g;
 }
 
+constexpr int WINO_BG_MAXL = 9;
+constexpr int WINO_BG_KEYS = WINO_BG_MAXL * WINO_BG_MAXL * WINO_BG_MAXL * WINO_BG_MAXL;
+
+__global__ __launch_bounds__(256) void wino_bg_z1_kernel(const unsigned char *__restrict__ valid, int B, int X, int Y, int Z, int TX, int TY,
+                                                         unsigned char *__restrict__ z1) {
+  const int tile = blockIdx.x * 4 + (threadIdx.x >> 6), lane = threadIdx.x & 63;
+  if (tile >= B * TX * TY) return;
+  const int ty = tile % TY, tx = (tile / TY) % TX, b = tile / (TY * TX);
+  const int x = 6 * tx - 1 + (lane >> 3), y = 6 * ty - 1 + (lane & 7);
+  bool any = false;
+  if ((unsigned)x < (unsigned)X && (unsigned)y < (unsigned)Y) {
+    const unsigned char *v = valid + (((size_t)b * X + x) * Y + y) * Z;
+    for (int z = 0; z < Z; ++z) any |= v[z] != 0;
+  }
+  const bool wave_any = __ballot(any) != 0;
+  if (lane == 0) z1[tile] = wave_any ? 0 : 1;
+}
+
+struct WinoBgPlanP {
+  const unsigned char *z1;
+  unsigned char *scratch;
+  int *layers;
+  int B, TX, TY, nl, lstride, nb;
+  int zo[WINO_BG_MAXL];
+};
+constexpr int WINO_BG_LDS_TILES = 16384;
+
+__device__ __forceinline__ int wino_bg_scan(const int v, int *wsum, int *total) {
+  const int lane = threadIdx.x & 63, wave = threadIdx.x >> 6;
+  int incl = v;
+#pragma unroll
+  for (int o = 1; o < 64; o <<= 1) {
+    const int x = __shfl_up(incl, o);
+    if (lane >= o) incl += x;
+  }
+  __syncthreads();
+  if (lane == 63) wsum[wave] = incl;
+  __syncthreads();
+  int base = 0, tot = 0;
+#pragma unroll
+  for (int w = 0; w < 16; ++w) {
+    const int x = wsum[w];
+    base += w < wave ? x : 0;
+    tot += x;
+  }
+  *total = tot;
+  return base + incl - v;
+}
+
+__global__ __launch_bounds__(1024) void wino_bg_plan_kernel(const WinoBgPlanP p) {
+  __shared__ int rep[WINO_BG_KEYS];
+  __shared__ int wsum[16];
+  __shared__ unsigned char qlds[2][WINO_BG_LDS_TILES];
+  const int tid = threadIdx.x, l = blockIdx.x;
+  const int n = p.B * p.TX * p.TY;
+  const int chunk = (n + 1023) / 1024;
+  const int t0 = min(tid * chunk, n), t1 = min(t0 + chunk, n);
+  unsigned char *qa = n <= WINO_BG_LDS_TILES ? qlds[0] : p.scratch + (size_t)(2 * l) * p.nb;
+  unsigned char *qb = n <= WINO_BG_LDS_TILES ? qlds[1] : p.scratch + (size_t)(2 * l + 1) * p.nb;
+  const int cap = l, LK = cap + 1, K = LK * LK * LK * LK;
+  int *blk = p.layers + (size_t)l * p.lstride, *list = blk + WINO_BG_HDR, *src = list + n;
+  auto key = [&](int t) {
+    const int ty = t % p.TY, tx = (t / p.TY) % p.TX;
+    return ((min(tx, cap) * LK + min(p.TX - 1 - tx, cap)) * LK + min(ty, cap)) * LK + min(p.TY - 1 - ty, cap);
+  };
+  for (int t = tid; t < n; t += 1024) qa[t] = p.z1[t];
+  for (int k = tid; k < K; k += 1024) rep[k] = 0x7fffffff;
+  __syncthreads();
+  for (int e = 0; e < l; ++e) {
+    for (int t = tid; t < n; t += 1024) {
+      const int ty = t % p.TY, tx = (t / p.TY) % p.TX, b0 = t - tx * p.TY - ty;
+      int q = 1;
+      for (int dx = -1; dx <= 1; ++dx)
+        for (int dy = -1; dy <= 1; ++dy) {
+          const int xx = tx + dx, yy = ty + dy;
+          if ((unsigned)xx < (unsigned)p.TX && (unsigned)yy < (unsigned)p.TY) q &= qa[b0 + xx * p.TY + yy];
+        }
+      qb[t] = (unsigned char)q;
+    }
+    __syncthreads();
+    unsigned char *sw = qa; qa = qb; qb = sw;
+  }
+  int cnt = 0;
+  for (int t = t0; t < t1; ++t) {
+    if (!qa[t]) ++cnt;
+    else atomicMin(&rep[key(t)], t);
+  }
+  int na;
+  int o = wino_bg_scan(cnt, wsum, &na);
+  for (int t = t0; t < t1; ++t)
+    if (!qa[t]) { list[o] = t; src[t] = o; ++o; }
+  const int kchunk = (K + 1023) / 1024, k0 = min(tid * kchunk, K), k1 = min(k0 + kchunk, K);
+  cnt = 0;
+  for (int k = k0; k < k1; ++k) cnt += rep[k] != 0x7fffffff;
+  int nk;
+  int r = wino_bg_scan(cnt, wsum, &nk);
+  for (int k = k0; k < k1; ++k)
+    if (rep[k] != 0x7fffffff) { list[na + r] = rep[k]; rep[k] = r; ++r; }
+  __syncthreads();
+  for (int t = t0; t < t1; ++t)
+    if (qa[t]) src[t] = na + rep[key(t)];
+  if (tid == 0) { blk[0] = na + nk; blk[1] = (na + nk) * p.zo[l]; blk[2] = na; blk[3] = nk; }
+}
+
+struct WinoBgLayout { int64_t z1, scratch, layers, lstride, total, nb; int n; };
+WinoBgLayout wino_bg_layout(int B, int TX, int TY, int n_layers) {
+  WinoBgLayout L;
+  L.n = B * TX * TY;
+  L.nb = ivx_align_up((int64_t)L.n, 256);
+  L.z1 = 0; L.scratch = L.nb;
+  L.layers = L.nb + (L.n <= WINO_BG_LDS_TILES ? 0 : 2 * (int64_t)WINO_BG_MAXL * L.nb);
+  L.lstride = ivx_align_up((int64_t)(WINO_BG_HDR + 2 * (int64_t)L.n) * 4, 256) / 4;
+  L.total = L.layers + (int64_t)n_layers * L.lstride * 4;
+  return L;
+}
 unsigned wino_blocks(int64_t items) {
   const int64_t b = (items + 255) / 256;
   return (unsigned)(b < 1 ? 1 : (b > (1 << 20) ? (1 << 20) : b));
@@ -707,6 +831,7 @@
   p->relu = d->relu; p->res_mode = d->res_mode; p->res_after_act = d->res_after_act;
   p->post_scale = d->post_scale == 0.f ? 1.0f : d->post_scale;
   p->pmax = nullptr;
+  p->bg = nullptr;
 #ifdef IVX_CONV_TIMELINE
   p->tl = g_wino_timeline;
 #endif
@@ -717,14 +842,24 @@
 }
 }
 
+static int wino_bg_check(const ivx_conv_desc *d, int32_t tile, const void *bg, const char *who) {
+  if (bg && !ivx_conv_winograd_bg_supported(d, tile)) {
+    ivx_set_error("%s: the layer does not take the background form (ivx_conv_winograd_bg_supported)", who);
+    return IVX_ERR_UNSUPPORTED;
+  }
+  return IVX_OK;
+}
+
 static int wino_input_impl(const ivx_conv_desc *d, int32_t tile, const void *in, void *workspace, int64_t workspace_bytes,
-                           const float *partials, int32_t n_partials, ivx_stream_t stream) {
+                           const float *partials, int32_t n_partials, const int32_t *bg, ivx_stream_t stream) {
   WinoDims w;
   WinoP p;
   float dummy;
   IVX_REQUIRE(in, "ivx_conv_winograd_input: null argument");
   int rc = wino_setup(d, tile, in, nullptr, nullptr, &dummy, &dummy, workspace, workspace_bytes, &w, &p, "ivx_conv_winograd_input");
   if (rc != IVX_OK) return rc;
+  if ((rc = wino_bg_check(d, tile, bg, "ivx_conv_winograd_input")) != IVX_OK) return rc;
+  p.bg = bg;
   if (d->wino_operands == IVX_F16_PAIR) {
     static const bool one_wg = !(getenv("IVX_WINO_AMAX_ONE_WG") && atoi(getenv("IVX_WINO_AMAX_ONE_WG")) == 0);
     const bool write_form = partials && n_partials <= 65536 && one_wg;
@@ -762,17 +897,23 @@
 
 extern "C" int ivx_conv_winograd_input(const ivx_conv_desc *d, int32_t tile, const void *in, void *workspace, int64_t workspace_bytes,
                                        ivx_stream_t stream) {
-  return wino_input_impl(d, tile, in, workspace, workspace_bytes, nullptr, 0, stream);
+  return wino_input_impl(d, tile, in, workspace, workspace_bytes, nullptr, 0, nullptr, stream);
 }
 
 extern "C" int ivx_conv_winograd_input_amax(const ivx_conv_desc *d, int32_t tile, const void *in, void *workspace, int64_t workspace_bytes,
                                             const float *partials, int32_t n_partials, ivx_stream_t stream) {
   IVX_REQUIRE(!partials || n_partials > 0, "ivx_conv_winograd_input_amax: partials without a count");
-  return wino_input_impl(d, tile, in, workspace, workspace_bytes, partials, n_partials, stream);
-}
-
-extern "C" int ivx_conv_winograd_gemm(const ivx_conv_desc *d, int32_t tile, const float *u, void *workspace, int64_t workspace_bytes,
-                                      ivx_stream_t stream) {
+  return wino_input_impl(d, tile, in, workspace, workspace_bytes, partials, n_partials, nullptr, stream);
+}
+
+extern "C" int ivx_conv_winograd_input_bg(const ivx_conv_desc *d, int32_t tile, const void *in, void *workspace, int64_t workspace_bytes,
+                                          const float *partials, int32_t n_partials, const int32_t *bg, ivx_stream_t stream) {
+  IVX_REQUIRE(!partials || n_partials > 0, "ivx_conv_winograd_input_bg: partials without a count");
+  return wino_input_impl(d, tile, in, workspace, workspace_bytes, partials, n_partials, bg, stream);
+}
+
+static int wino_gemm_impl(const ivx_conv_desc *d, int32_t tile, const float *u, void *workspace, int64_t workspace_bytes, const int32_t *bg,
+                          ivx_stream_t stream) {
   WinoDims w;
   WinoP p;
   float dummy;
@@ -783,11 +924,22 @@
   const long long el = d->wino_operands == IVX_F16_PAIR ? 2 : 1;
   g.in_dtype = d->wino_operands;
   const unsigned *us = p.hdr ? reinterpret_cast<const unsigned *>(u + (int64_t)w.n2 * d->Cout * d->KW * d->Cin + 1) : nullptr;
+  if ((rc = wino_bg_check(d, tile, bg, "ivx_conv_winograd_gemm")) != IVX_OK) return rc;
   rc = ivx_conv_grouped_launch(&g, w.n2, p.V, el * w.v_stride, u, el * d->Cout * d->KW * d->Cin, p.Mw, w.m_stride, (hipStream_t)stream, us,
-                               p.hdr ? const_cast<unsigned *>(p.hdr) + 1 : nullptr);
+                               p.hdr ? const_cast<unsigned *>(p.hdr) + 1 : nullptr, bg ? bg + 1 : nullptr);
   if (rc != IVX_OK) return rc;
   IVX_CHECK_LAUNCH("ivx_conv_winograd_gemm");
   return IVX_OK;
+}
+
+extern "C" int ivx_conv_winograd_gemm(const ivx_conv_desc *d, int32_t tile, const float *u, void *workspace, int64_t workspace_bytes,
+                                      ivx_stream_t stream) {
+  return wino_gemm_impl(d, tile, u, workspace, workspace_bytes, nullptr, stream);
+}
+
+extern "C" int ivx_conv_winograd_gemm_bg(const ivx_conv_desc *d, int32_t tile, const float *u, void *workspace, int64_t workspace_bytes,
+                                         const int32_t *bg, ivx_stream_t stream) {
+  return wino_gemm_impl(d, tile, u, workspace, workspace_bytes, bg, stream);
 }
 
 extern "C" int ivx_conv_winograd_fused_supported(const ivx_conv_desc *d, int32_t tile) {
@@ -863,7 +1015,7 @@
 }
 
 static int wino_output_impl(const ivx_conv_desc *d, int32_t tile, const float *scale, const float *shift, const void *res, void *out,
-                            void *workspace, int64_t workspace_bytes, float *partials, ivx_stream_t stream) {
+                            void *workspace, int64_t workspace_bytes, float *partials, const int32_t *bg, ivx_stream_t stream) {
   WinoDims w;
   WinoP p;
   float dummy;
@@ -871,7 +1023,9 @@
   IVX_REQUIRE(!d || d->res_mode == 0 || res, "ivx_conv_winograd_output: res_mode set but res is NULL");
   int rc = wino_setup(d, tile, &dummy, scale, shift, res, out, workspace, workspace_bytes, &w, &p, "ivx_conv_winograd_output");
   if (rc != IVX_OK) return rc;
+  if ((rc = wino_bg_check(d, tile, bg, "ivx_conv_winograd_output")) != IVX_OK) return rc;
   p.pmax = partials;
+  p.bg = bg;
   if (tile == 2)
     hipLaunchKernelGGL((wino_output_kernel<2, 4>), dim3(wino_blocks(w.m_elems / 4)), dim3(256), 0, (hipStream_t)stream, p);
   else if (tile == 4)
@@ -898,12 +1052,69 @@
 
 extern "C" int ivx_conv_winograd_output(const ivx_conv_desc *d, int32_t tile, const float *scale, const float *shift, const void *res,
                                         void *out, void *workspace, int64_t workspace_bytes, ivx_stream_t stream) {
-  return wino_output_impl(d, tile, scale, shift, res, out, workspace, workspace_bytes, nullptr, stream);
+  return wino_output_impl(d, tile, scale, shift, res, out, workspace, workspace_bytes, nullptr, nullptr, stream);
 }
 
 extern "C" int ivx_conv_winograd_output_amax(const ivx_conv_desc *d, int32_t tile, const float *scale, const float *shift, const void *res,
                                              void *out, void *workspace, int64_t workspace_bytes, float *partials, ivx_stream_t stream) {
-  return wino_output_impl(d, tile, scale, shift, res, out, workspace, workspace_bytes, partials, stream);
+  return wino_output_impl(d, tile, scale, shift, res, out, workspace, workspace_bytes, partials, nullptr, stream);
+}
+
+extern "C" int ivx_conv_winograd_output_bg(const ivx_conv_desc *d, int32_t tile, const float *scale, const float *shift, const void *res,
+                                           void *out, void *workspace, int64_t workspace_bytes, float *partials, const int32_t *bg,
+                                           ivx_stream_t stream) {
+  return wino_output_impl(d, tile, scale, shift, res, out, workspace, workspace_bytes, partials, bg, stream);
+}
+
+extern "C" int ivx_conv_winograd_bg_supported(const ivx_conv_desc *d, int32_t tile) {
+  WinoDims w;
+  if (tile != 6 || !d || d->pd != 1 || d->ph != 1 || !ivx_conv_winograd_supported(d, tile)) return 0;
+  if (wino_dims(d, tile, &w, "ivx_conv_winograd_bg_supported") != IVX_OK) return 0;
+  ivx_conv_desc g = wino_group_desc(d, w);
+  g.in_dtype = d->wino_operands;
+  return ivx_conv_grouped_rows_dev_ok(&g, w.n2);
+}
+
+extern "C" int64_t ivx_conv_winograd_bg_bytes(const ivx_conv_desc *d, int32_t n_layers) {
+  WinoDims w;
+  if (wino_dims(d, 6, &w, "ivx_conv_winograd_bg_bytes") != IVX_OK) return -1;
+  IVX_REQUIRE(n_layers >= 1 && n_layers <= WINO_BG_MAXL, "ivx_conv_winograd_bg_bytes: 1 .. %d layers", WINO_BG_MAXL) ;
+  return wino_bg_layout(d->B, w.TX, w.TY, n_layers).total;
+}
+
+extern "C" int64_t ivx_conv_winograd_bg_layer_offset(const ivx_conv_desc *d, int32_t layer) {
+  WinoDims w;
+  if (wino_dims(d, 6, &w, "ivx_conv_winograd_bg_layer_offset") != IVX_OK) return -1;
+  IVX_REQUIRE(layer >= 0 && layer < WINO_BG_MAXL, "ivx_conv_winograd_bg_layer_offset: bad layer");
+  const WinoBgLayout L = wino_bg_layout(d->B, w.TX, w.TY, layer + 1);
+  return L.layers + (int64_t)layer * L.lstride * 4;
+}
+
+extern "C" int ivx_conv_winograd_bg_plan(const ivx_conv_desc *d, const uint8_t *valid, int32_t n_layers, const int32_t *out_slices, void *block,
+                                         int64_t block_bytes, ivx_stream_t stream) {
+  WinoDims w;
+  int rc = wino_dims(d, 6, &w, "ivx_conv_winograd_bg_plan");
+  if (rc != IVX_OK) return rc;
+  IVX_REQUIRE(valid && out_slices && block, "ivx_conv_winograd_bg_plan: null argument");
+  IVX_REQUIRE(n_layers >= 1 && n_layers <= WINO_BG_MAXL, "ivx_conv_winograd_bg_plan: 1 .. %d layers", WINO_BG_MAXL);
+  IVX_REQUIRE(d->pd == 1 && d->ph == 1, "ivx_conv_winograd_bg_plan: the chain's layers pad x and y by 1");
+  const WinoBgLayout L = wino_bg_layout(d->B, w.TX, w.TY, n_layers);
+  if (block_bytes < L.total) {
+    ivx_set_error("ivx_conv_winograd_bg_plan: block too small (%lld < %lld); size it with ivx_conv_winograd_bg_bytes", (long long)block_bytes,
+                  (long long)L.total);
+    return IVX_ERR_WORKSPACE;
+  }
+  char *base = (char *)block;
+  WinoBgPlanP p;
+  p.z1 = (const unsigned char *)(base + L.z1); p.scratch = (unsigned char *)(base + L.scratch);
+  p.layers = (int *)(base + L.layers);
+  p.B = d->B; p.TX = w.TX; p.TY = w.TY; p.nl = n_layers; p.lstride = (int)L.lstride; p.nb = (int)L.nb;
+  for (int l = 0; l < WINO_BG_MAXL; ++l) p.zo[l] = l < n_layers ? out_slices[l] : 0;
+  hipLaunchKernelGGL(wino_bg_z1_kernel, dim3((unsigned)((L.n + 3) / 4)), dim3(256), 0, (hipStream_t)stream, valid, d->B, d->D, d->H, d->W, w.TX, w.TY,
+                     (unsigned char *)(base + L.z1));
+  hipLaunchKernelGGL(wino_bg_plan_kernel, dim3((unsigned)n_layers), dim3(1024), 0, (hipStream_t)stream, p);
+  IVX_CHECK_LAUNCH("ivx_conv_winograd_bg_plan");
+  return IVX_OK;
 }
 
 extern "C" int ivx_conv_winograd_fwd(const ivx_conv_desc *d, int32_t tile, const void *in, const float *u, const float *scale,
diff --git a/imvoxelnet_amd/ops.py b/imvoxelnet_amd/ops.py
--- a/imvoxelnet_amd/ops.py
+++ b/imvoxelnet_amd/ops.py
@@ -210,8 +210,29 @@
 winograd_trace = None
 
 
+def winograd_bg_plan(valid, x_shape, Cout, out_slices, wgt_layout=1, operands=IVX_F16_PAIR):
+    B, X, Y, Z, Cin = x_shape
+    if tuple(valid.shape) != (B, X, Y, Z) or not valid.is_cuda or not valid.is_contiguous() or valid.element_size() != 1:
+        raise ValueError('valid must be a contiguous [B,X,Y,Z] one-byte device tensor')
+    d = _wino_desc(B, X, Y, Z, Cin, Cout, 3, 1, (1, 1, 1), False, wgt_layout, operands=operands)
+    L = _lib.lib()
+    nl = len(out_slices)
+    nb = L.ivx_conv_winograd_bg_bytes(C.byref(d), nl)
+    if nb < 0:
+        check(-1, 'ivx_conv_winograd_bg_bytes')
+    block = torch.zeros((nb,), device=valid.device, dtype=torch.uint8)
+    zo = (C.c_int32 * nl)(*[int(z) for z in out_slices])
+    check(L.ivx_conv_winograd_bg_plan(C.byref(d), _ptr(valid), nl, zo, _ptr(block), nb, _stream()), 'ivx_conv_winograd_bg_plan')
+    n = B * ((X + 5) // 6) * ((Y + 5) // 6)
+    views = []
+    for l in range(nl):
+        off = L.ivx_conv_winograd_bg_layer_offset(C.byref(d), l)
+        views.append(block[off:off + 4 * (4 + 2 * n)].view(torch.int32))
+    return block, views
+
+
 def conv_winograd_fwd(x, u, scale=None, shift=None, kw=3, stride_w=1, padding=(1, 1, 1), relu=False, res=None, out=None,
-                      wgt_layout=0, res_after_act=False, post_scale=1.0, operands=0, amax_in=None, want_amax=False, fused=False):
+                      wgt_layout=0, res_after_act=False, post_scale=1.0, operands=0, amax_in=None, want_amax=False, fused=False, bg=None):
     _chk(x, 'x')
     _chk(u, 'u')
     B, D, H, W, Cin = x.shape
@@ -254,6 +275,20 @@
                                              _stream()), 'ivx_conv_winograd_input_amax')
         check(L.ivx_conv_winograd_gemm_output_amax(C.byref(d), tile, _ptr(u), _ptr(scale), _ptr(shift), _ptr(res), _ptr(out), _ptr(ws), wsb, _ptr(part),
                                                    _stream()), 'ivx_conv_winograd_gemm_output_amax')
+        return (out, part) if want_amax else out
+    if bg is not None:
+        if not L.ivx_conv_winograd_bg_supported(C.byref(d), tile):
+            raise ValueError('this layer does not take the background form (ivx_conv_winograd_bg_supported)')
+        part = None
+        if want_amax:
+            part = torch.empty((L.ivx_conv_winograd_output_blocks(C.byref(d), tile),), device=x.device, dtype=torch.float32)
+        if amax_in is not None:
+            _chk(amax_in, 'amax_in')
+        check(L.ivx_conv_winograd_input_bg(C.byref(d), tile, _ptr(x), _ptr(ws), wsb, _ptr(amax_in), 0 if amax_in is None else amax_in.numel(),
+                                           _ptr(bg), _stream()), 'ivx_conv_winograd_input_bg')
+        check(L.ivx_conv_winograd_gemm_bg(C.byref(d), tile, _ptr(u), _ptr(ws), wsb, _ptr(bg), _stream()), 'ivx_conv_winograd_gemm_bg')
+        check(L.ivx_conv_winograd_output_bg(C.byref(d), tile, _ptr(scale), _ptr(shift), _ptr(res), _ptr(out), _ptr(ws), wsb, _ptr(part),
+                                            _ptr(bg), _stream()), 'ivx_conv_winograd_output_bg')
         return (out, part) if want_amax else out
     if amax_in is not None or want_amax:
         part = None
diff --git a/include/imvoxel.h b/include/imvoxel.h
--- a/include/imvoxel.h
+++ b/include/imvoxel.h
@@ -148,6 +148,17 @@
 int ivx_conv_winograd_gemm_output_amax(const ivx_conv_desc *d, int32_t tile, const float *u, const float *scale, const float *shift,
                                        const void *res, void *out, void *workspace, int64_t workspace_bytes, float *partials,
                                        ivx_stream_t stream);
+int ivx_conv_winograd_bg_supported(const ivx_conv_desc *d, int32_t tile);
+int64_t ivx_conv_winograd_bg_bytes(const ivx_conv_desc *d, int32_t n_layers);
+int64_t ivx_conv_winograd_bg_layer_offset(const ivx_conv_desc *d, int32_t layer);
+int ivx_conv_winograd_bg_plan(const ivx_conv_desc *d, const uint8_t *valid, int32_t n_layers, const int32_t *out_slices, void *block,
+                              int64_t block_bytes, ivx_stream_t stream);
+int ivx_conv_winograd_input_bg(const ivx_conv_desc *d, int32_t tile, const void *in, void *workspace, int64_t workspace_bytes,
+                               const float *partials, int32_t n_partials, const int32_t *bg, ivx_stream_t stream);
+int ivx_conv_winograd_gemm_bg(const ivx_conv_desc *d, int32_t tile, const float *u, void *workspace, int64_t workspace_bytes,
+                              const int32_t *bg, ivx_stream_t stream);
+int ivx_conv_winograd_output_bg(const ivx_conv_desc *d, int32_t tile, const float *scale, const float *shift, const void *res, void *out,
+                                void *workspace, int64_t workspace_bytes, float *partials, const int32_t *bg, ivx_stream_t stream);
 
 
 int ivx_dcn_im2col_fwd(const float *x, const float *offset_mask, int32_t B, int32_t H, int32_t W, int32_t C, int32_t kh,
```

After: 280.9 images/s, median of 6. +7.0%, better.
